# ARM-software/astc-encoder

Measured on AMD Instinct MI355X. Metric: Mtexels/s + PSNR-dB, 8192x8192 RGBA8 LDR 6x6 -medium, higher is better.
Workload: dtype f32

## Files before the change

astc-encoder_amd/csrc/astc_tables.h:

```cpp
#pragma once
#if !defined(__HIPCC_RTC__)
#include <stdint.h>
#include <stddef.h>
#else
typedef unsigned char uint8_t; typedef signed char int8_t; typedef unsigned short uint16_t; typedef short int16_t;
typedef unsigned int uint32_t; typedef int int32_t; typedef unsigned long uint64_t; typedef long int64_t;
typedef unsigned long size_t; typedef unsigned long uintptr_t; typedef long ptrdiff_t;
#define offsetof(type, member) __builtin_offsetof(type, member)
#endif

#if defined(__HIPCC__)
	#define ASTC_HD __host__ __device__
#else
	#define ASTC_HD
#endif

namespace astcd {

constexpr int MAX_TEXELS       = 216;
constexpr int MAX_WEIGHTS      = 64;
constexpr int PLANE2_OFFSET    = 32;
constexpr int MAX_PARTITIONS   = 4;
constexpr int MAX_PARTITIONINGS = 1024;
constexpr int MAX_KMEANS_TEXELS = 64;
constexpr int MAX_BLOCK_MODES  = 2048;
constexpr int MAX_DECIMATION_MODES = 87;
constexpr int MAX_TRIAL_CANDIDATES = 8;
constexpr int MAX_PARTITIONING_CANDIDATES = 8;
constexpr int MAX_ANGULAR_QUANT = 7;
constexpr int ANGULAR_STEPS = 32;
constexpr int SINCOS_STEPS  = 64;
constexpr float ERROR_CALC_DEFAULT = 1e30f;

enum {
	FMT_LUMINANCE = 0, FMT_LUMINANCE_DELTA = 1, FMT_HDR_LUMINANCE_LARGE_RANGE = 2,
	FMT_HDR_LUMINANCE_SMALL_RANGE = 3, FMT_LUMINANCE_ALPHA = 4, FMT_LUMINANCE_ALPHA_DELTA = 5,
	FMT_RGB_SCALE = 6, FMT_HDR_RGB_SCALE = 7, FMT_RGB = 8, FMT_RGB_DELTA = 9,
	FMT_RGB_SCALE_ALPHA = 10, FMT_HDR_RGB = 11, FMT_RGBA = 12, FMT_RGBA_DELTA = 13,
	FMT_HDR_RGB_LDR_ALPHA = 14, FMT_HDR_RGBA = 15
};

enum {
	QUANT_2 = 0, QUANT_3, QUANT_4, QUANT_5, QUANT_6, QUANT_8, QUANT_10, QUANT_12, QUANT_16,
	QUANT_20, QUANT_24, QUANT_32, QUANT_40, QUANT_48, QUANT_64, QUANT_80, QUANT_96, QUANT_128,
	QUANT_160, QUANT_192, QUANT_256
};

constexpr uint32_t MODE_DESC_BYTES = 16 + 2 * 32;
constexpr uint32_t MODE_WEIGHT_BYTES = 68;
constexpr uint32_t MODE_Q2U_BYTES = 12 * 32;
constexpr uint32_t FMT_QUANT_ROWS = 17;
ASTC_HD inline uint32_t fmt_comb_cols(uint32_t partition_limit) { return partition_limit <= 1 ? 0u : partition_limit == 2 ? 7u : partition_limit == 3 ? 10u : 13u; }
ASTC_HD inline uint32_t fmt_scratch_bytes(uint32_t partition_limit)
{
	uint32_t P = partition_limit < 1 ? 1u : partition_limit > 4 ? 4u : partition_limit;
	return P * FMT_QUANT_ROWS * 4 * 4 + P * FMT_QUANT_ROWS * 4 + FMT_QUANT_ROWS * fmt_comb_cols(P) * (4 + 2);
}
constexpr uint32_t ANG_PAIR_STRIDE = 9;
ASTC_HD inline uint32_t uni_region_bytes(uint32_t texel_count, uint32_t partition_limit)
{
	const uint32_t Tp = (texel_count + 3u) & ~3u;
	uint32_t bytes = 64 * ANG_PAIR_STRIDE * 4;
	if (8u * (MODE_DESC_BYTES + 64u + Tp * 4) > bytes) bytes = 8u * (MODE_DESC_BYTES + 64u + Tp * 4);
	if (fmt_scratch_bytes(partition_limit) > bytes) bytes = fmt_scratch_bytes(partition_limit);
	if (5 * Tp * 4 > bytes) bytes = 5 * Tp * 4;
	return (bytes + 15u) & ~15u;
}

enum { SYM_BTYPE_ERROR = 0, SYM_BTYPE_CONST_F16 = 1, SYM_BTYPE_CONST_U16 = 2, SYM_BTYPE_NONCONST = 3 };

struct BlockMode {
	uint16_t mode_index;
	uint8_t  decimation_mode;
	uint8_t  quant_mode;
	uint8_t  weight_bits;
	uint8_t  is_dual_plane;
	uint8_t  pad[2];
};

struct ModeStatic {
	uint32_t tw_off;
	uint32_t tcf_off;
	uint16_t dwi_off[2];
	uint16_t lh_off[2];
	uint8_t  taps;
	uint8_t  weights;
	uint8_t  quant_mode;
	uint8_t  weight_bits;
	uint8_t  is_dual_plane;
	uint8_t  pad[3];
};

struct DecimationMode {
	int8_t   maxprec_1plane;
	int8_t   maxprec_2planes;
	uint16_t refprec_1plane;
	uint16_t refprec_2planes;
	uint16_t dwi_offset[3];
	uint16_t lowhigh_offset[3];
};

struct DwiTap8 { uint32_t w[4]; };
struct DwiSlot {
	uint32_t wt_off;
	uint32_t wc_off;
	uint16_t refprec;
	uint8_t  weight_count;
	uint8_t  taps;
	uint8_t  flags;
	uint8_t  dm;
	uint8_t  set;
	uint8_t  index;
};

constexpr int DWI_MAX_CHUNKS = 15;
struct DwiOrderDir {
	uint32_t list_off;
	uint16_t chunk_start[DWI_MAX_CHUNKS + 1];
	uint16_t chunks;
	uint16_t pad;
};

struct InfillSet {
	uint32_t tw_off;
	uint32_t tcf_off;
	uint16_t dwi_offset;
	uint16_t refprec;
	uint8_t  taps;
	uint8_t  direct;
	uint8_t  dm;
	uint8_t  plane;
};

struct DecimationInfo {
	uint8_t  texel_count;
	uint8_t  weight_count;
	uint8_t  max_texel_weight_count;
	uint8_t  weight_x;
	uint8_t  weight_y;
	uint8_t  max_weight_texel_count;
	uint8_t  realign_levels;
	uint8_t  realign_slots;
	uint32_t off_texel_weights;
	uint32_t off_texel_contribs_int;
	uint32_t off_texel_contribs_f;
	uint32_t off_weight_texel_count;
	uint32_t off_weight_texels;
	uint32_t off_weight_contribs;
	uint32_t off_texel_contrib_for_weight;
	uint32_t off_realign_order;
	uint32_t off_realign_counts;
	uint32_t table_bytes;
	uint32_t off_realign_later;
	uint32_t realign_speculative;
	uint32_t pad[2];
};
static_assert(sizeof(DecimationInfo) == 64, "DecimationInfo is staged as one 64-byte record");
constexpr int REALIGN_LATER_MAX = 16;
#ifndef ASTC_REALIGN_SPEC_MIN
#define ASTC_REALIGN_SPEC_MIN 2
#endif
constexpr int REALIGN_SPECULATIVE_MIN_LEVELS = ASTC_REALIGN_SPEC_MIN;

struct PartitionHeader {
	uint16_t partition_index;
	uint8_t  partition_count;
	uint8_t  pad;
	uint8_t  texel_count[4];
};

struct QuantXfer {
	uint8_t  quant_to_unquant[32];
	uint8_t  scramble_map[32];
	uint16_t prev_next_values[65];
	uint16_t pad;
};

constexpr uint32_t CTX_CONFIG_BACK = 256;
constexpr uint32_t CTX_LAYOUT_BACK = 1024;

struct TableRoot {
	uint8_t  dim_x, dim_y, texel_count, dim_z;
	uint32_t block_mode_count_1plane_always;
	uint32_t block_mode_count_1plane_selected;
	uint32_t block_mode_count_1plane_2plane_selected;
	uint32_t decimation_mode_count_always;
	uint32_t decimation_mode_count_selected;
	uint32_t partitioning_count_selected[4];
	uint32_t partition_stride;
	uint32_t off_block_modes;
	uint32_t off_decimation_modes;
	uint32_t off_decimation_infos;
	uint32_t off_partitions[4];
	uint32_t off_coverage[4];
	uint32_t off_kmeans_texels;
	uint32_t off_color_unquant_to_uquant;
	uint32_t off_color_uquant_to_pquant;
	uint32_t off_quant_xfer;
	uint32_t off_quant_mode_table;
	uint32_t off_quant_mode_by_bits;
	uint32_t off_mode_levels;
	uint32_t off_integer_of_trits;
	uint32_t off_integer_of_quints;
	uint32_t off_sin_table;
	uint32_t off_cos_table;
	uint32_t off_cos_sin_table;
	uint32_t off_dm_by_weights;
	uint32_t off_mode_static;
	uint32_t max_decimation_table_bytes;
	uint32_t max_weight_texel_rows;
	uint32_t realign_rt_floats;
	uint32_t max_weights[2];
	uint32_t dwi_total_floats[2];
	uint32_t off_dwi_owner[2];
	uint32_t off_dwi_slots[2];
	uint32_t off_infill_sets[2];
	uint32_t dwi_sets[2];
	uint32_t dwi_used_sets[2][12];
	uint32_t lowhigh_floats[2];
	uint32_t off_dwi_order[2];
	uint32_t dwi_sets_per_chunk;
	uint32_t max_partitionings;
	uint32_t total_bytes;
};

struct DeviceConfig {
	int32_t  profile;
	uint32_t flags;
	float    cw[4];
	float    rgbm_m_scale;
	uint32_t tune_partition_count_limit;
	uint32_t tune_partition_index_limit[3];
	uint32_t tune_refinement_limit;
	uint32_t tune_candidate_limit;
	uint32_t tune_partitioning_candidate_limit[3];
	float    tune_db_limit;
	float    tune_mse_overshoot;
	float    tune_partition_early_out_limit_factor[2];
	float    tune_2plane_early_out_limit_correlation;
	float    tune_search_mode0_enable;
	uint32_t debug_dup_stage;
};

struct ImageDesc {
	const void* data;
	uint32_t dim_x, dim_y;
	uint32_t data_type;
	uint32_t swz[4];
	uint32_t blocks_x, blocks_y;
	uint32_t use_fast_load;
	const float* alpha_avg;
	uint32_t a_scale_radius;
	uint32_t dim_z, blocks_z;
	uint32_t fast_load_slice0;
	const uint32_t* list;
};

struct ImageSetEntryDesc {
	ImageDesc img;
	uint8_t* out;
};

}
```

astc-encoder_amd/csrc/backend.h:

```cpp
#pragma once
#include <stddef.h>
#include <stdint.h>
#include <atomic>
#include <vector>
#include "astc_tables.h"
#include "image_set.h"
#include "mip_filter.h"
#include "mip_post.h"

namespace astcd {

struct Backend;

struct CompressJob {
	const void* const* host_slices;
	const void* device_data;
	uint32_t dim_x, dim_y, dim_z;
	uint32_t data_type;
	uint32_t swz[4];
	uint8_t* host_out;
	uint8_t* device_out;
	void*    stream;
	float*   kernel_ms;
	uint32_t a_scale_radius;
	const std::atomic<int>* cancel_flag;
	void (*progress)(float);
	uint32_t fast_load_slice0;
	uint32_t halo_above, halo_below;
	const uint32_t* device_list;
	uint32_t list_count;
};

struct DecompressJob {
	const uint8_t* host_blocks;
	size_t   block_bytes;
	void* const* host_slices;
	uint32_t dim_x, dim_y, dim_z;
	uint32_t data_type;
	uint32_t swz[4];
};

struct DecompressDeviceJob {
	const uint8_t* device_blocks;
	void*    device_image;
	uint32_t dim_x, dim_y, dim_z;
	uint32_t data_type;
	uint32_t swz[4];
	void*    stream;
};

inline size_t texel_bytes(uint32_t data_type) { return data_type == 0 ? 4 : data_type == 1 ? 8 : 16; }

struct BlockGrid {
	uint32_t x, y, z;
	uint32_t dim_z;
	size_t count() const { return (size_t)x * y * z; }
};
template <class Job> inline BlockGrid block_grid(const TableRoot& root, const Job& job)
{
	const uint32_t dim_z = job.dim_z ? job.dim_z : 1u;
	return { (job.dim_x + root.dim_x - 1) / root.dim_x, (job.dim_y + root.dim_y - 1) / root.dim_y, (dim_z + root.dim_z - 1) / root.dim_z, dim_z };
}

inline bool uses_fast_load(const TableRoot& root, int32_t profile, const CompressJob& job)
{
	const bool identity = job.swz[0] == 0 && job.swz[1] == 1 && job.swz[2] == 2 && job.swz[3] == 3;
	return identity && profile < 2 && job.data_type == 0 && root.dim_z == 1;
}

inline ImageDesc image_desc(const TableRoot& root, int32_t profile, const CompressJob& job, const void* data)
{
	const BlockGrid g = block_grid(root, job);
	ImageDesc img;
	img.data = data;
	img.dim_x = job.dim_x; img.dim_y = job.dim_y; img.dim_z = g.dim_z;
	img.data_type = job.data_type;
	for (int i = 0; i < 4; i++) img.swz[i] = job.swz[i];
	img.blocks_x = g.x; img.blocks_y = g.y; img.blocks_z = g.z;
	img.use_fast_load = uses_fast_load(root, profile, job) ? 1 : 0;
	img.fast_load_slice0 = job.fast_load_slice0;
	img.alpha_avg = nullptr;
	img.a_scale_radius = job.a_scale_radius;
	img.list = job.device_list;
	return img;
}

struct CompressSetJob {
	const CompressJob* entries;
	uint32_t count;
	void*    stream;
	float*   kernel_ms;
	const std::atomic<int>* cancel_flag;
	void (*progress)(float);
	const struct MipChainJob* generate;
};

struct MipChainJob {
	const void* device_image;
	uint32_t dim_x, dim_y, dim_z, kind, data_type, level_count;
	uint32_t srgb;
	uint8_t* device_levels;
	size_t texels_offset[MIP_MAX_LEVELS];
	void* stream;
	uint32_t post_flags;
	float alpha_cutoff;
	uint32_t cover_t;
	float cover_hi, cover_lo;
	uint32_t filter_kind, filter_edge;
	uint32_t weight;
};

struct ResizeJob {
	const void* device_image;
	void* device_out;
	uint32_t dim_x, dim_y, dim_z, out_x, out_y, out_z, kind, data_type, srgb;
	uint32_t filter_kind, filter_edge, weight;
	void* stream;
	float* kernel_ms;
};

struct DecompressSetJob {
	const DecompressDeviceJob* entries;
	uint32_t count;
	void*    stream;
};

struct CompareJob {
	const void* device_a; uint32_t type_a;
	const void* device_b; uint32_t type_b;
	size_t texels;
	void* stream;
	double* sums;
	int hdr, fstop_lo, fstop_hi;
};
constexpr int METRIC_SUMS_HOST = 18;

struct QualityEntryJob {
	DecompressDeviceJob decode;
	const void* device_original; uint32_t original_type;
	double* device_block_errors;
};
struct QualitySetJob {
	const QualityEntryJob* entries;
	uint32_t count;
	void* stream;
	double* sums;
	int hdr, fstop_lo, fstop_hi;
};

Backend* backend_create(const uint8_t* blob, size_t blob_bytes, const DeviceConfig& cfg, int* status);
void backend_destroy(Backend* b);
int backend_device_count(const Backend* b);
int backend_compress(Backend* b, const CompressJob& job);
int backend_decompress(Backend* b, const DecompressJob& job);
int backend_decompress_device(Backend* b, const DecompressDeviceJob& job);
int backend_compare(Backend* b, const CompareJob& job);
int backend_compress_set(Backend* b, const CompressSetJob& job);
int backend_decompress_set(Backend* b, const DecompressSetJob& job);
int backend_compare_blocks_set(Backend* b, const QualitySetJob& job);
struct SelectJob {
	const double* device_block_errors;
	uint32_t dim_x, dim_y, dim_z;
	uint32_t blocks;
	double weight[4], max_mse;
	uint32_t* device_list;
	void* stream;
	uint32_t* count;
};
struct AdaptiveJob {
	CompressJob strong;
	DecompressDeviceJob decode;
	double weight[4], max_mse;
	double* device_block_errors;
	uint32_t* selected; uint32_t* replaced;
	float* kernel_ms_strong; float* kernel_ms_other;
};
int backend_select_blocks(Backend* b, const SelectJob& job);
int backend_adaptive_reserve(Backend* b, const void* device_image, const void* device_out, const void* device_block_errors, size_t blocks);
int backend_adaptive_refine(Backend* b, const AdaptiveJob& job);
int backend_generate_mips(Backend* b, const MipChainJob& job);
int backend_resize(Backend* b, const ResizeJob& job);
void backend_log(const char* fmt, ...) __attribute__((format(printf, 1, 2)));
const char* backend_name();
void backend_set_log_callback(void (*callback)(const char* message));


struct KernelLaunch {
	const uint8_t* d_tab;
	uint32_t lds_bytes;
	ImageDesc img;
	uint8_t* d_out;
	uint32_t first, count;
	void* stream;
	unsigned long long* d_prof;
	const ImageSetTable* d_set;
};

int astc_kernel_prepare_ldr(const TableRoot& root, const DeviceConfig& cfg, uint32_t* lds_bytes, void* layout_out, uint32_t* layout_bytes);
int astc_kernel_prepare_hdr(const TableRoot& root, const DeviceConfig& cfg, uint32_t* lds_bytes, void* layout_out, uint32_t* layout_bytes);
int astc_kernel_launch_ldr(const KernelLaunch& k);
int astc_kernel_launch_hdr(const KernelLaunch& k);
int astc_kernel_prepare_ldr64(const TableRoot& root, const DeviceConfig& cfg, uint32_t* lds_bytes, void* layout_out, uint32_t* layout_bytes);
int astc_kernel_prepare_hdr64(const TableRoot& root, const DeviceConfig& cfg, uint32_t* lds_bytes, void* layout_out, uint32_t* layout_bytes);
int astc_kernel_launch_ldr64(const KernelLaunch& k);
int astc_kernel_launch_hdr64(const KernelLaunch& k);
constexpr int ASTC_PREPARE_NOT_THIS_CONTEXT = -1;
#define ASTC_DECLARE_KERNEL_VARIANT(tag) \
	int astc_kernel_prepare_##tag(const TableRoot& root, const DeviceConfig& cfg, uint32_t* lds_bytes, void* layout_out, uint32_t* layout_bytes); \
	int astc_kernel_launch_##tag(const KernelLaunch& k);
ASTC_DECLARE_KERNEL_VARIANT(ldr_6x6m)
ASTC_DECLARE_KERNEL_VARIANT(ldr_8x8t)
ASTC_DECLARE_KERNEL_VARIANT(hdr_6x6m)
#undef ASTC_DECLARE_KERNEL_VARIANT
const char* backend_kernel_name(const Backend* b);
int backend_specialize(Backend* b);

constexpr size_t ALPHA_LDS_LIMIT = 160u * 1024u;
constexpr uint32_t ALPHA_TILE_ROWS_2D = 32;
struct AlphaLaunch {
	const void* d_image;
	float* d_averages;
	uint32_t dim_x, dim_y, dim_z, data_type, swz_a, radius;
	float* d_scratch; uint32_t scratch_workgroups;
	void* stream;
};
size_t astc_alpha_scratch_bytes(uint32_t dim_x, uint32_t dim_y, uint32_t dim_z, uint32_t radius, uint32_t* workgroups);
int astc_alpha_launch(const AlphaLaunch& a);

struct DecodeLaunch {
	const uint8_t* d_blocks;
	void* d_image;
	const void* d_tables;
	uint32_t dim_x, dim_y, dim_z, data_type, swz[4];
	uint32_t block_x, block_y, block_z, profile;
	void* stream;
};
int astc_decode_launch(const DecodeLaunch& d);
size_t astc_decode_set_bytes(uint32_t count);
uint32_t astc_decode_set_build(void* out, const DecodeLaunch* entries, uint32_t count);
int astc_decode_set_launch(const void* d_table, uint32_t runs, void* stream);
size_t astc_decode_tables_bytes();
void astc_decode_tables_build(void* out, uint32_t block_x, uint32_t block_y, uint32_t block_z);

struct QualityLaunch {
	DecodeLaunch decode;
	const void* d_original; uint32_t original_type;
	double* d_block_errors;
};
size_t astc_quality_set_bytes(uint32_t count);
size_t astc_quality_scratch_doubles();
uint32_t astc_quality_set_build(void* out, const QualityLaunch* entries, uint32_t count);
int astc_quality_set_launch(const void* h_table, const void* d_table, double* d_partials, double* d_sums, int hdr, int fstop_lo, int fstop_hi, void* stream);

struct SelectLaunch {
	const double* d_errors;
	uint32_t dim_x, dim_y, dim_z, block_x, block_y, block_z, blocks;
	double weight[4], max_mse;
	uint32_t* d_list;
	uint32_t* d_counts;
	void* stream;
};
size_t astc_select_scratch_words(size_t blocks);
size_t astc_select_total_word(size_t blocks);
int astc_select_launch(const SelectLaunch& s);
struct MergeLaunch {
	const uint32_t* d_list; const uint32_t* d_count;
	uint32_t blocks;
	uint32_t max_count;
	const double* d_strong_errors; double* d_base_errors;
	const uint8_t* d_strong; uint8_t* d_out;
	double weight[4];
	uint32_t* d_replaced;
	void* stream;
};
int astc_merge_launch(const MergeLaunch& m);

int astc_mip_launch(const MipChainJob& job, const void* d_srgb, void* stream);
size_t astc_mip_srgb_table_bytes();
void astc_mip_srgb_tables_build(void* out);
int astc_mip_weighted_launch(const MipChainJob& job, const void* d_srgb, void* stream);
int astc_mip_filter_table_build(const MipChainJob& job, std::vector<uint8_t>& out);
int astc_mip_filter_launch(const MipChainJob& job, const void* d_table, const void* d_srgb, void* stream);
int astc_mip_filter_weighted_launch(const MipChainJob& job, const void* d_table, const void* d_srgb, void* stream);
int astc_mip_cube_launch(const MipChainJob& job, const void* d_table, const void* d_srgb, void* stream);
size_t astc_mip_post_scratch_bytes(const MipChainJob& job);
int astc_mip_post_launch(const MipChainJob& job, void* d_scratch, void* stream);

int astc_resize_table_build(const ResizeJob& job, std::vector<uint8_t>& out);
int astc_resize_launch(const ResizeJob& job, const void* d_table, const void* d_srgb, void* stream);

struct CompareLaunch {
	const void* d_a; uint32_t type_a;
	const void* d_b; uint32_t type_b;
	size_t texels;
	double* d_sums;
	void* stream;
	int hdr, fstop_lo, fstop_hi;
};
int astc_compare_launch(const CompareLaunch& c);
size_t astc_compare_scratch_doubles();

}
```

astc-encoder_amd/csrc/backend_hip.hip:

```cpp
#include "backend.h"
#include "kernel_jit.h"
#include "mip_resample.h"

#include <hip/hip_runtime.h>
#include <chrono>
#include <cstdarg>
#include <cstdio>
#include <sched.h>
#include <atomic>
#include <cstdlib>
#include <cstring>
#include <condition_variable>
#include <functional>
#include <mutex>
#include <new>
#include <thread>
#include <type_traits>
#include <utility>
#include <vector>

namespace astcd {

struct SlotWorker {
	std::mutex mu;
	std::mutex state_mu;
	std::condition_variable wake, done_cv;
	std::function<void()> task;
	bool has_task = false, done = true, quit = false, bound = false;
	std::thread thread;
	bool started = false;
};

struct DeviceSlot {
	int device = 0;
	uint8_t* d_base = nullptr;
	uint8_t* d_tab = nullptr;
	uint8_t* d_dectab = nullptr;
	const double* d_srgb = nullptr;
	hipStream_t stream = nullptr;
	hipStream_t copy_stream = nullptr;
	hipEvent_t ev0 = nullptr, ev1 = nullptr, ev_copy[2] = {}, ev_band = nullptr, ev_done[3] = {}, ev_out[2] = {};
	hipEvent_t ev_gen = nullptr;
	uint8_t* h_in[2] = {}; size_t h_in_cap = 0;
	uint8_t* h_out[2] = {}; size_t h_out_cap = 0;
	void* d_image = nullptr; size_t image_cap = 0;
	uint8_t* d_out = nullptr; size_t out_cap = 0;
	float* d_alpha = nullptr; size_t alpha_cap = 0;
	float* d_alpha_scratch = nullptr; size_t alpha_scratch_cap = 0;
	uint8_t* d_mip_post = nullptr; size_t mip_post_cap = 0;
	uint8_t* d_mip_filter = nullptr; size_t mip_filter_cap = 0;
	std::vector<uint8_t> h_mip_filter;
	uint8_t* d_set = nullptr; size_t set_cap = 0;
	std::vector<uint8_t> h_set;
	unsigned long long* d_prof = nullptr;
	size_t trace_cap = 0;
	double* d_sums = nullptr;
	double* d_quality = nullptr; size_t quality_cap = 0;
	double* d_quality_sums = nullptr; size_t quality_sums_cap = 0;
	uint32_t* d_select = nullptr; size_t select_cap = 0;
	uint8_t* d_adaptive = nullptr; size_t adaptive_cap = 0;
	hipEvent_t ev_adapt[2] = {};
	std::mutex busy;
	std::vector<int> local_cpus;
	SlotWorker* worker = nullptr;
	hipModule_t jit_module = nullptr;
	hipFunction_t jit_fn = nullptr;
	bool jit_tried = false;
};

struct Backend {
	std::vector<DeviceSlot*> slots;
	std::vector<DeviceSlot*> extra;
	std::mutex slots_mu;
	std::vector<uint8_t> full;
	size_t dectab_offset;
	size_t srgb_offset;
	DeviceConfig cfg;
	uint32_t lds_bytes;
	bool hdr;
	TableRoot root;
	int variant;
	JitKernel* jit;
	JitMode jit_mode;
	std::atomic<unsigned long long> blocks_done;
	unsigned long long jit_lazy_blocks;
	std::atomic<bool> jit_active;
};

constexpr size_t ALLOC_SLACK = 4096;
constexpr size_t BAND_MIN_BLOCKS = (size_t)1 << 18;
#if defined(ASTC_TRACE)
constexpr size_t TRACE_WORDS_PER_BLOCK_HOST = 1024;
#endif

static std::atomic<void (*)(const char*)> g_log_callback{nullptr};
void backend_set_log_callback(void (*cb)(const char*)) { g_log_callback.store(cb); }
static void log_msg(const char* fmt, ...) __attribute__((format(printf, 1, 2)));
static void log_msg(const char* fmt, ...)
{
	void (*cb)(const char*) = g_log_callback.load();
	static const bool to_stderr = []() { const char* e = getenv("ASTCENC_AMD_LOG"); return e && strcmp(e, "stderr") == 0; }();
	if (!cb && !to_stderr) return;
	char line[512];
	va_list ap;
	va_start(ap, fmt);
	vsnprintf(line, sizeof(line), fmt, ap);
	va_end(ap);
	if (cb) cb(line);
	else fprintf(stderr, "astcenc_amd: %s\n", line);
}

void backend_log(const char* fmt, ...)
{
	char line[512];
	va_list ap;
	va_start(ap, fmt);
	vsnprintf(line, sizeof(line), fmt, ap);
	va_end(ap);
	log_msg("%s", line);
}

#define HIP_TRY(expr, fail) do { hipError_t e_ = (expr); if (e_ != hipSuccess) { \
	log_msg("%s -> %s", #expr, hipGetErrorString(e_)); fail; } } while (0)

const char* backend_name() { return "hip:gfx950"; }

namespace {

struct DeviceGuard {
	int saved; bool ok;
	DeviceGuard() : saved(0), ok(hipGetDevice(&saved) == hipSuccess) {}
	~DeviceGuard() { if (ok) (void)hipSetDevice(saved); }
};

template <class T> int grow(T*& buf, size_t& cap, size_t need)
{
	if (cap >= need) return 0;
	if (buf) (void)hipFree(buf);
	buf = nullptr; cap = 0;
	HIP_TRY(hipMalloc(reinterpret_cast<void**>(&buf), need + ALLOC_SLACK), return 1);
	cap = need;
	return 0;
}
int grow_pinned(uint8_t* (&pair)[2], size_t& cap, size_t need)
{
	if (cap >= need) return 0;
	for (uint8_t*& h : pair) { if (h) (void)hipHostFree(h); h = nullptr; }
	cap = 0;
	for (uint8_t*& h : pair) HIP_TRY(hipHostMalloc(reinterpret_cast<void**>(&h), need, hipHostMallocDefault), return 1);
	cap = need;
	return 0;
}

struct KernelVariant {
	const char* name;
	bool fixed, hdr, small;
	int (*prepare)(const TableRoot&, const DeviceConfig&, uint32_t*, void*, uint32_t*);
	int (*launch)(const KernelLaunch&);
};
const KernelVariant kernel_variants[] = {
	{ "astc_compress_blocks_ldr_6x6m", true, false, true, astc_kernel_prepare_ldr_6x6m, astc_kernel_launch_ldr_6x6m },
	{ "astc_compress_blocks_ldr_8x8t", true, false, true, astc_kernel_prepare_ldr_8x8t, astc_kernel_launch_ldr_8x8t },
	{ "astc_compress_blocks_hdr_6x6m", true, true, true, astc_kernel_prepare_hdr_6x6m, astc_kernel_launch_hdr_6x6m },
	{ "astc_compress_blocks_ldr64", false, false, true, astc_kernel_prepare_ldr64, astc_kernel_launch_ldr64 },
	{ "astc_compress_blocks_hdr64", false, true, true, astc_kernel_prepare_hdr64, astc_kernel_launch_hdr64 },
	{ "astc_compress_blocks_ldr", false, false, false, astc_kernel_prepare_ldr, astc_kernel_launch_ldr },
	{ "astc_compress_blocks_hdr", false, true, false, astc_kernel_prepare_hdr, astc_kernel_launch_hdr },
};
int kernel_prepare(Backend* b, uint32_t* lds_bytes, void* layout_out, uint32_t* layout_bytes)
{
	if (b->variant >= 0) return kernel_variants[b->variant].prepare(b->root, b->cfg, lds_bytes, layout_out, layout_bytes);
	const bool small = b->root.texel_count <= 64;
	const char* want = getenv("ASTCENC_AMD_KERNEL");
	const bool generic_only = want && strcmp(want, "generic") == 0;
	for (int i = 0; i < (int)(sizeof(kernel_variants) / sizeof(kernel_variants[0])); i++)
	{
		const KernelVariant& v = kernel_variants[i];
		if (v.hdr != b->hdr || v.small != small || (v.fixed && generic_only)) continue;
		const int rc = v.prepare(b->root, b->cfg, lds_bytes, layout_out, layout_bytes);
		if (rc == ASTC_PREPARE_NOT_THIS_CONTEXT) continue;
		if (rc == 0) b->variant = i;
		return rc;
	}
	return (int)hipErrorInvalidDeviceFunction;
}
int kernel_launch(const Backend* b, const DeviceSlot* s, const KernelLaunch& k)
{
	if (s->jit_fn)
	{
		KernelLaunch a = k;
		void* args[] = { &a.d_tab, &a.img, &a.d_out, &a.first, &a.count, &a.d_prof, &a.d_set };
		return (int)hipModuleLaunchKernel(s->jit_fn, k.count, 1, 1, 64, 1, 1, k.lds_bytes, static_cast<hipStream_t>(k.stream), args, nullptr);
	}
	return kernel_variants[b->variant].launch(k);
}

bool jit_self_check(Backend* b, DeviceSlot* s, hipFunction_t fn)
{
	const uint32_t bsx = b->root.dim_x, bsy = b->root.dim_y, bsz = b->root.dim_z;
	const uint32_t nbx = bsz > 1 ? 16u : 48u, nby = bsz > 1 ? 16u : 48u, nbz = bsz > 1 ? 8u : 1u;
	const uint32_t dim_x = nbx * bsx - 1u, dim_y = nby * bsy - 1u, dim_z = bsz > 1 ? nbz * bsz - 1u : 1u;
	const size_t texels = (size_t)dim_x * dim_y * dim_z, nblocks = (size_t)nbx * nby * nbz;
	std::vector<uint8_t> img(texels * 4);
	uint32_t rng = 0x9E3779B1u;
	auto tri = [](uint32_t v) { const uint32_t m = v & 511u; return (int)(m < 256u ? m : 511u - m); };
	for (uint32_t z = 0; z < dim_z; z++)
		for (uint32_t y = 0; y < dim_y; y++)
			for (uint32_t x = 0; x < dim_x; x++)
			{
				const uint32_t tile = (x / bsx + 3u * (y / bsy) + 5u * (z / bsz) + y / (3u * bsy)) % 9u;
				uint8_t* px = &img[(((size_t)z * dim_y + y) * dim_x + x) * 4];
				int grey = 0;
				for (int ch = 0; ch < 4; ch++)
				{
					rng = rng * 1664525u + 1013904223u;
					const int noise = (int)(rng >> 24);
					int v = (int)((x * (3u + ch) + y * (7u - ch) + z * 11u) & 255u);
					if (tile == 1) v += (noise & 15) - 6;
					else if (tile == 2) v += (noise & 63) - 24;
					else if (tile == 3) v = noise;
					else if (tile == 4) v = ((x + ch) ^ (y >> 1)) & 2 ? 220 - 20 * ch : 30 + 25 * ch;
					else if (tile == 5) v = 40 + 50 * ch;
					else if (tile == 6 || tile == 7)
					{
						if (ch == 0) grey = (3 * tri(x + 2u * y + 5u * z) + tri((3u * x + 512u - y) >> 1)) / 4 + noise % 21 - 10;
						v = ch < 3 ? grey : 192 + tri((x >> 1) + (y >> 2)) / 4 + noise % 7 - 3;
					}
					else if (tile == 8) v = tri(x * (2u + ch) + y * (5u - ch) + z * 3u);
					if (ch == 3 && tile != 3 && tile != 2 && tile != 7) v = 255;
					px[ch] = (uint8_t)(v < 0 ? 0 : v > 255 ? 255 : v);
				}
			}
	void* d_img = nullptr;
	uint8_t* d_out = nullptr;
	bool ok = hipMalloc(&d_img, img.size() + ALLOC_SLACK) == hipSuccess && hipMalloc(reinterpret_cast<void**>(&d_out), 2 * nblocks * 16 + ALLOC_SLACK) == hipSuccess;
	std::vector<uint8_t> out(2 * nblocks * 16);
	if (ok)
	{
		CompressJob job;
		memset(&job, 0, sizeof(job));
		job.dim_x = dim_x; job.dim_y = dim_y; job.dim_z = dim_z;
		for (int i = 0; i < 4; i++) job.swz[i] = (uint32_t)i;
		KernelLaunch k;
		k.d_tab = s->d_tab; k.lds_bytes = b->lds_bytes; k.d_prof = nullptr; k.d_set = nullptr; k.stream = s->stream;
		k.first = 0; k.count = (uint32_t)nblocks;
		k.img = image_desc(b->root, b->cfg.profile, job, d_img);
		ok = hipMemcpyAsync(d_img, img.data(), img.size(), hipMemcpyHostToDevice, s->stream) == hipSuccess;
		k.d_out = d_out;
		ok = ok && kernel_variants[b->variant].launch(k) == 0;
		k.d_out = d_out + nblocks * 16;
		void* args[] = { &k.d_tab, &k.img, &k.d_out, &k.first, &k.count, &k.d_prof, &k.d_set };
		ok = ok && hipModuleLaunchKernel(fn, k.count, 1, 1, 64, 1, 1, k.lds_bytes, s->stream, args, nullptr) == hipSuccess;
		ok = ok && hipMemcpyAsync(out.data(), d_out, out.size(), hipMemcpyDeviceToHost, s->stream) == hipSuccess;
		ok = ok && hipStreamSynchronize(s->stream) == hipSuccess;
		if (!ok) (void)hipGetLastError();
	}
	if (d_img) (void)hipFree(d_img);
	if (d_out) (void)hipFree(d_out);
	return ok && memcmp(out.data(), out.data() + nblocks * 16, nblocks * 16) == 0;
}

void slot_adopt_jit(Backend* b, DeviceSlot* s)
{
	if (!b->jit || s->jit_tried || jit_state(b->jit) != JIT_READY) return;
	s->jit_tried = true;
	size_t bytes = 0;
	const void* code = jit_code(b->jit, &bytes);
	hipModule_t mod = nullptr;
	hipFunction_t fn = nullptr;
	if (hipModuleLoadData(&mod, code) != hipSuccess || hipModuleGetFunction(&fn, mod, JIT_ENTRY_POINT) != hipSuccess)
	{
		(void)hipGetLastError();
		if (mod) (void)hipModuleUnload(mod);
		log_msg("run-time build %s does not load on device %d: the generic build stays", jit_kernel_name(b->jit), s->device);
		return;
	}
	const char* check = getenv("ASTCENC_AMD_JIT_SELF_CHECK");
	if (!(check && strcmp(check, "0") == 0) && !jit_self_check(b, s, fn))
	{
		(void)hipModuleUnload(mod);
		log_msg("run-time build %s does not reproduce the generic build's bytes on the self-check image: the generic build stays", jit_kernel_name(b->jit));
		return;
	}
	s->jit_module = mod;
	s->jit_fn = fn;
	b->jit_active.store(true);
}

void worker_stop(SlotWorker* w)
{
	if (!w) return;
	if (w->started)
	{
		{ std::lock_guard<std::mutex> g(w->state_mu); w->quit = true; }
		w->wake.notify_one();
		w->thread.join();
	}
	delete w;
}

void slot_destroy(DeviceSlot* s)
{
	if (!s) return;
	worker_stop(s->worker);
	s->worker = nullptr;
	(void)hipSetDevice(s->device);
	if (s->d_image) (void)hipFree(s->d_image);
	if (s->d_out) (void)hipFree(s->d_out);
	if (s->d_alpha) (void)hipFree(s->d_alpha);
	if (s->d_alpha_scratch) (void)hipFree(s->d_alpha_scratch);
	if (s->d_mip_post) (void)hipFree(s->d_mip_post);
	if (s->d_mip_filter) (void)hipFree(s->d_mip_filter);
	if (s->d_set) (void)hipFree(s->d_set);
	if (s->d_sums) (void)hipFree(s->d_sums);
	if (s->d_quality) (void)hipFree(s->d_quality);
	if (s->d_quality_sums) (void)hipFree(s->d_quality_sums);
	if (s->d_select) (void)hipFree(s->d_select);
	if (s->d_adaptive) (void)hipFree(s->d_adaptive);
	for (hipEvent_t e : s->ev_adapt) if (e) (void)hipEventDestroy(e);
	if (s->d_prof) (void)hipFree(s->d_prof);
	for (int i = 0; i < 2; i++) { if (s->h_in[i]) (void)hipHostFree(s->h_in[i]); if (s->h_out[i]) (void)hipHostFree(s->h_out[i]); }
	for (hipEvent_t e : { s->ev_copy[0], s->ev_copy[1], s->ev_band, s->ev_done[0], s->ev_done[1], s->ev_done[2], s->ev_out[0], s->ev_out[1], s->ev0, s->ev1, s->ev_gen })
		if (e) (void)hipEventDestroy(e);
	if (s->copy_stream) (void)hipStreamDestroy(s->copy_stream);
	if (s->stream) (void)hipStreamDestroy(s->stream);
	if (s->jit_module) (void)hipModuleUnload(s->jit_module);
	if (s->d_base) (void)hipFree(s->d_base);
	delete s;
}

static std::vector<int> device_local_cpus(int device)
{
	std::vector<int> cpus;
	char bus[64] = { 0 };
	if (hipDeviceGetPCIBusId(bus, (int)sizeof(bus), device) != hipSuccess) return cpus;
	for (char* p = bus; *p; p++) if (*p >= 'A' && *p <= 'F') *p = (char)(*p - 'A' + 'a');
	char path[160];
	snprintf(path, sizeof(path), "/sys/bus/pci/devices/%s/local_cpulist", bus);
	FILE* f = fopen(path, "r");
	if (!f) return cpus;
	char line[1024] = { 0 };
	if (fgets(line, (int)sizeof(line), f))
	{
		for (char* p = line; *p && *p != '\n'; )
		{
			char* end = nullptr;
			long a = strtol(p, &end, 10);
			if (end == p) break;
			long bnd = a;
			p = end;
			if (*p == '-') { bnd = strtol(p + 1, &end, 10); p = end; }
			for (long c = a; c <= bnd && c < 4096; c++) cpus.push_back((int)c);
			if (*p == ',') p++;
		}
	}
	fclose(f);
	return cpus;
}

static void bind_worker_to_device(const DeviceSlot* s)
{
	static const bool enabled = []() { const char* e = getenv("ASTCENC_AMD_NUMA_BIND"); return !(e && e[0] == '0'); }();
	if (!enabled || s->local_cpus.empty()) return;
	cpu_set_t allowed, want;
	CPU_ZERO(&want);
	if (sched_getaffinity(0, sizeof(allowed), &allowed) != 0) return;
	int n = 0;
	for (int c : s->local_cpus) if (c < CPU_SETSIZE && CPU_ISSET(c, &allowed)) { CPU_SET(c, &want); n++; }
	if (n > 0) (void)sched_setaffinity(0, sizeof(want), &want);
}

static bool worker_run(DeviceSlot* s, std::function<void()> task)
{
	SlotWorker* w = s->worker;
	if (!w) return false;
	if (!w->mu.try_lock()) return false;
	if (!w->started)
	{
		try
		{
			w->thread = std::thread([w, s]()
			{
				bind_worker_to_device(s);
				std::unique_lock<std::mutex> lk(w->state_mu);
				for (;;)
				{
					w->wake.wait(lk, [w]() { return w->has_task || w->quit; });
					if (w->quit) return;
					std::function<void()> t = std::move(w->task);
					w->has_task = false;
					lk.unlock();
					t();
					lk.lock();
					w->done = true;
					w->done_cv.notify_all();
				}
			});
			w->started = true;
		}
		catch (...) { w->mu.unlock(); return false; }
	}
	{
		std::lock_guard<std::mutex> g(w->state_mu);
		w->task = std::move(task);
		w->has_task = true;
		w->done = false;
	}
	w->wake.notify_one();
	return true;
}
static void worker_wait(DeviceSlot* s)
{
	SlotWorker* w = s->worker;
	{
		std::unique_lock<std::mutex> lk(w->state_mu);
		w->done_cv.wait(lk, [w]() { return w->done; });
	}
	w->mu.unlock();
}

DeviceSlot* slot_create(Backend* b, int device, int* status)
{
	DeviceSlot* s = new DeviceSlot();
	s->device = device;
#define SLOT_TRY(expr, code) HIP_TRY(expr, { slot_destroy(s); *status = code; return nullptr; })
	SLOT_TRY(hipSetDevice(device), 2);
	{
		uint8_t layout[CTX_LAYOUT_BACK - CTX_CONFIG_BACK]; uint32_t layout_bytes = 0, lds_bytes = 0;
		int prc = kernel_prepare(b, &lds_bytes, layout, &layout_bytes);
		if (prc != 0)
		{
			log_msg("kernel setup failed on device %d (hip error %d)", device, prc);
			slot_destroy(s); *status = 2; return nullptr;
		}
	}
	SLOT_TRY(hipMalloc(&s->d_base, b->full.size() + ALLOC_SLACK), 1);
	SLOT_TRY(hipMemcpy(s->d_base, b->full.data(), b->full.size(), hipMemcpyHostToDevice), 2);
	s->d_tab = s->d_base + CTX_LAYOUT_BACK;
	s->d_dectab = s->d_base + b->dectab_offset;
	s->d_srgb = reinterpret_cast<const double*>(s->d_base + b->srgb_offset);
	SLOT_TRY(hipStreamCreateWithFlags(&s->stream, hipStreamNonBlocking), 2);
	SLOT_TRY(hipStreamCreateWithFlags(&s->copy_stream, hipStreamNonBlocking), 2);
	SLOT_TRY(hipEventCreateWithFlags(&s->ev_copy[0], hipEventDisableTiming), 2);
	SLOT_TRY(hipEventCreateWithFlags(&s->ev_copy[1], hipEventDisableTiming), 2);
	SLOT_TRY(hipEventCreateWithFlags(&s->ev_band, hipEventDisableTiming), 2);
	for (int i = 0; i < 3; i++) SLOT_TRY(hipEventCreateWithFlags(&s->ev_done[i], hipEventDisableTiming), 2);
	for (int i = 0; i < 2; i++) SLOT_TRY(hipEventCreateWithFlags(&s->ev_out[i], hipEventDisableTiming), 2);
	SLOT_TRY(hipEventCreate(&s->ev0), 2);
	SLOT_TRY(hipEventCreate(&s->ev1), 2);
	SLOT_TRY(hipEventCreate(&s->ev_gen), 2);
#if defined(ASTC_PROFILE)
	enum { PS_COUNT = 40 };
	SLOT_TRY(hipMalloc(&s->d_prof, 2 * PS_COUNT * sizeof(unsigned long long)), 1);
	SLOT_TRY(hipMemset(s->d_prof, 0, 2 * PS_COUNT * sizeof(unsigned long long)), 2);
#endif
#undef SLOT_TRY
	s->local_cpus = device_local_cpus(device);
	slot_adopt_jit(b, s);
	*status = 0;
	return s;
}

std::vector<int> device_list(int ndev)
{
	std::vector<int> out;
	const char* env = getenv("ASTCENC_AMD_DEVICES");
	const bool all = env && strcmp(env, "all") == 0;
	if (env && *env && !all)
	{
		const char* p = env;
		while (*p)
		{
			char* e = nullptr;
			long v = strtol(p, &e, 10);
			if (e == p) break;
			if (v >= 0 && v < ndev) out.push_back((int)v);
			else log_msg("ASTCENC_AMD_DEVICES names device %ld, %d visible; ignored", v, ndev);
			p = e;
			while (*p == ',' || *p == ' ') p++;
		}
	}
	if (out.empty())
	{
		int cur = 0;
		if (hipGetDevice(&cur) != hipSuccess) cur = 0;
		out.push_back(cur);
		if (all) for (int d = 0; d < ndev; d++) if (d != cur) out.push_back(d);
	}
	return out;
}

DeviceSlot* slot_for_pointer(Backend* b, const void* ptr, int* status)
{
	*status = 0;
	hipPointerAttribute_t attr;
	memset(&attr, 0, sizeof(attr));
	if (!ptr || hipPointerGetAttributes(&attr, ptr) != hipSuccess)
	{
		(void)hipGetLastError();
		return b->slots[0];
	}
	for (DeviceSlot* s : b->slots) if (s->device == attr.device) return s;
	std::lock_guard<std::mutex> lk(b->slots_mu);
	for (DeviceSlot* s : b->extra) if (s->device == attr.device) return s;
	DeviceSlot* s = slot_create(b, attr.device, status);
	if (s) b->extra.push_back(s);
	return s;
}

bool pick_stream(const DeviceSlot* s, void* caller_stream, hipStream_t* out)
{
	*out = s->stream;
	if (!caller_stream) return true;
	hipStream_t stream = static_cast<hipStream_t>(caller_stream);
	hipDevice_t sdev = -1;
	if (hipStreamGetDevice(stream, &sdev) != hipSuccess) { (void)hipGetLastError(); sdev = s->device; }
	if ((int)sdev != s->device)
	{
		log_msg("the stream belongs to device %d, the buffers to device %d", (int)sdev, s->device);
		return false;
	}
	*out = stream;
	return true;
}

bool set_on_one_device(const DeviceSlot* s, const void* const* ptrs, size_t count)
{
	for (size_t i = 0; i < count; i++)
	{
		hipPointerAttribute_t attr;
		memset(&attr, 0, sizeof(attr));
		if (!ptrs[i] || hipPointerGetAttributes(&attr, ptrs[i]) != hipSuccess) { (void)hipGetLastError(); continue; }
		if (attr.device != s->device)
		{
			log_msg("image set entry %zu: a buffer of device %d, entry 0's are on device %d", i / 2, attr.device, s->device);
			return false;
		}
	}
	return true;
}

template <class Body> int run_locked(DeviceSlot* s, void* caller_stream, Body body)
{
	std::lock_guard<std::mutex> busy(s->busy);
	HIP_TRY(hipSetDevice(s->device), return 2);
	hipStream_t stream;
	if (!pick_stream(s, caller_stream, &stream)) return 3;
	return body(s, stream);
}

template <class Body> int run_on_owner(Backend* b, const void* owner, const void* const* same_device, size_t count, void* caller_stream, Body body)
{
	DeviceGuard guard;
	int st = 0;
	DeviceSlot* s = slot_for_pointer(b, owner, &st);
	if (!s) return st ? st : 2;
	if (!set_on_one_device(s, same_device, count)) return 3;
	return run_locked(s, caller_stream, body);
}

template <class Job> DecodeLaunch decode_launch(const Backend* b, const DeviceSlot* s, const Job& job, const uint8_t* d_blocks, void* d_image, hipStream_t stream)
{
	DecodeLaunch d;
	d.d_blocks = d_blocks;
	d.d_image = d_image;
	d.d_tables = s->d_dectab;
	d.dim_x = job.dim_x; d.dim_y = job.dim_y; d.dim_z = job.dim_z ? job.dim_z : 1u; d.data_type = job.data_type;
	for (int i = 0; i < 4; i++) d.swz[i] = job.swz[i];
	d.block_x = b->root.dim_x; d.block_y = b->root.dim_y; d.block_z = b->root.dim_z;
	d.profile = b->cfg.profile;
	d.stream = stream;
	return d;
}

struct Progress {
	std::mutex mu;
	size_t done, total;
	void (*callback)(float);
	void add(size_t n)
	{
		if (!callback) return;
		std::lock_guard<std::mutex> lk(mu);
		done += n;
		callback(100.0f * (float)done / (float)total);
	}
};

}

Backend* backend_create(const uint8_t* blob, size_t blob_bytes, const DeviceConfig& cfg, int* status)
{
	int ndev = 0;
	if (hipGetDeviceCount(&ndev) != hipSuccess || ndev == 0)
	{
		log_msg("no HIP device available; this library has no CPU fallback");
		*status = 2;
		return nullptr;
	}
	DeviceGuard guard;

	Backend* b = new Backend;
	b->cfg = cfg;
	memcpy(&b->root, blob, sizeof(TableRoot));
	b->hdr = cfg.profile >= 2;
	b->lds_bytes = 0;
	b->variant = -1;
	b->jit = nullptr; b->jit_mode = JIT_OFF; b->blocks_done.store(0); b->jit_active.store(false);
	b->jit_lazy_blocks = JIT_LAZY_BLOCKS;
	if (const char* e = getenv("ASTCENC_AMD_JIT_LAZY_BLOCKS")) { const long long v = strtoll(e, nullptr, 10); if (v >= 1) b->jit_lazy_blocks = (unsigned long long)v; }
	uint8_t layout[CTX_LAYOUT_BACK - CTX_CONFIG_BACK];
	uint32_t layout_bytes = 0;
	{
		int prc = kernel_prepare(b, &b->lds_bytes, layout, &layout_bytes);
		if (prc != 0)
		{
			log_msg("kernel setup failed (hip error %d)", prc);
			delete b; *status = 2; return nullptr;
		}
	}
	if (b->lds_bytes > 160 * 1024)
	{
		log_msg("block working set %u B; a CU has 160 KiB of LDS", b->lds_bytes);
		delete b; *status = 2; return nullptr;
	}

	b->dectab_offset = (CTX_LAYOUT_BACK + blob_bytes + 255) & ~(size_t)255;
	b->srgb_offset = (b->dectab_offset + astc_decode_tables_bytes() + 255) & ~(size_t)255;
	b->full.assign(b->srgb_offset + astc_mip_srgb_table_bytes(), 0);
	astc_decode_tables_build(b->full.data() + b->dectab_offset, b->root.dim_x, b->root.dim_y, b->root.dim_z);
	astc_mip_srgb_tables_build(b->full.data() + b->srgb_offset);
	memcpy(b->full.data(), layout, layout_bytes);
	static_assert(sizeof(DeviceConfig) <= 256, "DeviceConfig outgrew its slot");
	memcpy(b->full.data() + (CTX_LAYOUT_BACK - CTX_CONFIG_BACK), &b->cfg, sizeof(DeviceConfig));
	memcpy(b->full.data() + CTX_LAYOUT_BACK, blob, blob_bytes);

#if !defined(ASTC_TRACE) && !defined(ASTC_DUPSTAGE) && !defined(ASTC_PROFILE) && !defined(ASTC_LDS_PAD_ENV)
	{
		const char* want = getenv("ASTCENC_AMD_KERNEL");
		b->jit_mode = want && strcmp(want, "generic") == 0 ? JIT_OFF : jit_mode_from_environment();
		if (b->jit_mode != JIT_OFF && !kernel_variants[b->variant].fixed)
		{
			int dev = 0;
			hipDeviceProp_t prop;
			if (hipGetDevice(&dev) == hipSuccess && hipGetDeviceProperties(&prop, dev) == hipSuccess)
				b->jit = jit_acquire(layout, layout_bytes, b->cfg, b->root, b->hdr, prop.gcnArchName, [](const char* line) { log_msg("%s", line); });
			if (b->jit && b->jit_mode == JIT_EAGER) jit_start(b->jit);
			if (b->jit && b->jit_mode == JIT_SYNC) (void)jit_wait(b->jit);
		}
	}
#endif
	for (int device : device_list(ndev))
	{
		int st = 0;
		DeviceSlot* s = slot_create(b, device, &st);
		if (!s)
		{
			if (b->slots.empty()) { jit_release(b->jit); delete b; *status = st; return nullptr; }
			log_msg("device %d not usable, continuing with %zu device(s)", device, b->slots.size());
			continue;
		}
		if (!b->slots.empty()) s->worker = new (std::nothrow) SlotWorker();
		b->slots.push_back(s);
	}
	*status = 0;
	return b;
}

void backend_destroy(Backend* b)
{
	if (!b) return;
	DeviceGuard guard;
	for (DeviceSlot* s : b->slots) slot_destroy(s);
	for (DeviceSlot* s : b->extra) slot_destroy(s);
	jit_release(b->jit);
	delete b;
}

int backend_device_count(const Backend* b) { return (int)b->slots.size(); }
const char* backend_kernel_name(const Backend* b)
{
	if (b->jit && b->jit_active.load()) return jit_kernel_name(b->jit);
	return b->variant >= 0 ? kernel_variants[b->variant].name : "";
}

int backend_specialize(Backend* b)
{
	if (b->variant >= 0 && kernel_variants[b->variant].fixed) return 0;
	if (!b->jit || jit_wait(b->jit) != JIT_READY) return 1;
	DeviceGuard guard;
	for (DeviceSlot* s : b->slots)
	{
		std::lock_guard<std::mutex> busy(s->busy);
		if (hipSetDevice(s->device) == hipSuccess) slot_adopt_jit(b, s);
	}
	return b->jit_active.load() ? 0 : 1;
}

static void jit_count_blocks(Backend* b, DeviceSlot* s, size_t nblocks)
{
	slot_adopt_jit(b, s);
	if (b->jit && b->jit_mode == JIT_LAZY && b->blocks_done.fetch_add(nblocks) + nblocks >= b->jit_lazy_blocks) jit_start(b->jit);
}

static int alpha_prepass(DeviceSlot* s, hipStream_t stream, const void* d_image, float* d_averages, uint32_t dim_x, uint32_t rows,
                         uint32_t dim_z, uint32_t data_type, uint32_t swz_a, uint32_t radius)
{
	AlphaLaunch a;
	a.d_image = d_image; a.d_averages = d_averages;
	a.dim_x = dim_x; a.dim_y = rows; a.dim_z = dim_z; a.data_type = data_type;
	a.swz_a = swz_a; a.radius = radius; a.stream = stream;
	a.d_scratch = nullptr; a.scratch_workgroups = 0;
	const size_t scratch = astc_alpha_scratch_bytes(dim_x, rows, dim_z, radius, &a.scratch_workgroups);
	if (scratch == (size_t)-1)
	{
		log_msg("a_scale_radius %u needs more than 1 GiB of pre-pass scratch per tile: refused", radius);
		return 1;
	}
	if (scratch)
	{
		if (grow(s->d_alpha_scratch, s->alpha_scratch_cap, scratch) != 0) return 1;
		a.d_scratch = s->d_alpha_scratch;
	}
	int arc = astc_alpha_launch(a);
	if (arc != 0) { log_msg("alpha pre-pass launch failed (hip error %d)", arc); return 2; }
	return 0;
}

static void alpha_scratch_release(DeviceSlot* s, hipStream_t stream)
{
	if (s->alpha_scratch_cap > ((size_t)64 << 20))
	{
		(void)hipStreamSynchronize(stream);
		(void)hipFree(s->d_alpha_scratch);
		s->d_alpha_scratch = nullptr; s->alpha_scratch_cap = 0;
	}
}

struct ChunkLoop {
	KernelLaunch k;
	size_t nblocks, chunk;
	bool chunked;
	bool timed;
	const std::atomic<int>* cancel_flag;
	Progress* progress;
	std::function<int(size_t first, size_t n)> before_launch;
	std::function<int(size_t first, size_t n, size_t chunk_index, size_t prev_blocks)> after_launch;
	size_t launched, prev_blocks;
};

static int run_chunks(const Backend* b, DeviceSlot* s, ChunkLoop& L)
{
	const hipStream_t stream = static_cast<hipStream_t>(L.k.stream);
	if (L.timed) HIP_TRY(hipEventRecord(s->ev0, stream), return 2);
	L.launched = 0; L.prev_blocks = 0;
	size_t chunk_index = 0;
	for (size_t first = 0; first < L.nblocks; first += L.chunk, chunk_index++)
	{
		if (L.cancel_flag && L.cancel_flag->load(std::memory_order_relaxed)) break;
		size_t n = L.nblocks - first < L.chunk ? L.nblocks - first : L.chunk;
		if (L.before_launch && L.before_launch(first, n) != 0) return 2;
		KernelLaunch k = L.k;
		k.first = (uint32_t)first; k.count = (uint32_t)n;
		int lrc = kernel_launch(b, s, k);
		if (lrc != 0) { log_msg("kernel launch failed (hip error %d)", lrc); return 2; }
		L.launched = first + n;
		if (L.after_launch)
		{
			if (L.after_launch(first, n, chunk_index, L.prev_blocks) != 0) return 2;
		}
		else if (L.chunked)
		{
			HIP_TRY(hipEventRecord(s->ev_done[chunk_index % 3], stream), return 2);
			if (chunk_index > 0)
			{
				HIP_TRY(hipEventSynchronize(s->ev_done[(chunk_index - 1) % 3]), return 2);
				if (L.progress) L.progress->add(L.prev_blocks);
			}
		}
		L.prev_blocks = n;
	}
	if (L.timed) HIP_TRY(hipEventRecord(s->ev1, stream), return 2);
	return 0;
}

static int compress_pipeline(Backend* b, DeviceSlot* s, hipStream_t stream, const CompressJob& job, Progress* progress);

static int compress_on_slot(Backend* b, DeviceSlot* s, hipStream_t stream, const CompressJob& job, Progress* progress)
{
	const int rc = compress_pipeline(b, s, stream, job, progress);
	if (rc != 0)
	{
		(void)hipStreamSynchronize(s->copy_stream);
		(void)hipStreamSynchronize(s->stream);
	}
	return rc;
}

static int compress_pipeline(Backend* b, DeviceSlot* s, hipStream_t stream, const CompressJob& job, Progress* progress)
{
	const BlockGrid grid = block_grid(b->root, job);
	const uint32_t bsy = b->root.dim_y, dim_z = grid.dim_z, blocks_x = grid.x, blocks_y = grid.y;
	const size_t nblocks = job.device_list ? (size_t)job.list_count : grid.count();
	jit_count_blocks(b, s, nblocks);
	const size_t row_bytes = (size_t)job.dim_x * texel_bytes(job.data_type);
	const uint32_t halo_above = dim_z == 1 && job.a_scale_radius != 0 ? job.halo_above : 0u;
	const uint32_t halo_below = dim_z == 1 && job.a_scale_radius != 0 ? job.halo_below : 0u;
	const uint32_t rows_with_halo = job.dim_y + halo_above + halo_below;
	const size_t slice_bytes = rows_with_halo * row_bytes;
	const size_t image_bytes = slice_bytes * dim_z;
	const size_t out_bytes = grid.count() * 16;

	const void* d_image = job.device_data;
	uint8_t* d_out = job.device_out;

	if (job.host_slices)
	{
		if (grow(s->d_image, s->image_cap, image_bytes) != 0) return 1;
		d_image = s->d_image;
	}
	const bool banded = job.host_slices && job.host_out && dim_z == 1 && job.a_scale_radius == 0;
	if (job.host_slices && !banded)
	{
		for (uint32_t z = 0; z < dim_z; z++)
			HIP_TRY(hipMemcpyAsync(static_cast<uint8_t*>(s->d_image) + z * slice_bytes, job.host_slices[z], slice_bytes, hipMemcpyHostToDevice, stream), return 2);
	}
	if (job.host_out)
	{
		if (grow(s->d_out, s->out_cap, out_bytes) != 0) return 1;
		d_out = s->d_out;
	}
	if (!d_image || !d_out) return 2;

	ImageDesc img = image_desc(b->root, b->cfg.profile, job, static_cast<const uint8_t*>(d_image) + halo_above * row_bytes);
	if (job.a_scale_radius != 0)
	{
		if (grow(s->d_alpha, s->alpha_cap, (size_t)job.dim_x * rows_with_halo * sizeof(float)) != 0) return 1;
		const int arc = alpha_prepass(s, stream, d_image, s->d_alpha, job.dim_x, rows_with_halo, dim_z, job.data_type, job.swz[3], job.a_scale_radius);
		if (arc != 0) return arc;
		img.alpha_avg = s->d_alpha + (size_t)halo_above * job.dim_x;
		alpha_scratch_release(s, stream);
	}

	const bool chunked = (progress && progress->callback) || job.host_slices;
	size_t chunk = chunked ? (size_t)1 << 18 : nblocks;
	if (banded)
	{
		size_t rows = chunk / blocks_x;
		if (rows * 4 > blocks_y) rows = nblocks >= BAND_MIN_BLOCKS ? (blocks_y + 3) / 4 : blocks_y;
		if (rows < 1) rows = 1;
		chunk = rows * blocks_x;
	}
	if (banded)
	{
		const size_t band_rows = (chunk / blocks_x) * bsy;
		if (grow_pinned(s->h_in, s->h_in_cap, band_rows * row_bytes) != 0 || grow_pinned(s->h_out, s->h_out_cap, chunk * 16) != 0) return 1;
	}
	auto upload_band = [&](size_t band_first, size_t band_blocks) -> int {
		const size_t band = band_first / chunk;
		const size_t y0 = (band_first / blocks_x) * bsy;
		size_t y1 = ((band_first + band_blocks) / blocks_x) * bsy;
		if (y1 > job.dim_y) y1 = job.dim_y;
		if (band >= 2) HIP_TRY(hipEventSynchronize(s->ev_copy[band & 1]), return 2);
		memcpy(s->h_in[band & 1], static_cast<const uint8_t*>(job.host_slices[0]) + y0 * row_bytes, (y1 - y0) * row_bytes);
		HIP_TRY(hipMemcpyAsync(static_cast<uint8_t*>(s->d_image) + y0 * row_bytes, s->h_in[band & 1], (y1 - y0) * row_bytes, hipMemcpyHostToDevice, s->copy_stream), return 2);
		HIP_TRY(hipEventRecord(s->ev_copy[band & 1], s->copy_stream), return 2);
		return 0;
	};
	auto collect_band = [&](size_t band_first, size_t band_blocks) -> int {
		const size_t band = band_first / chunk;
		HIP_TRY(hipEventSynchronize(s->ev_out[band & 1]), return 2);
		memcpy(job.host_out + band_first * 16, s->h_out[band & 1], band_blocks * 16);
		if (progress) progress->add(band_blocks);
		return 0;
	};
#if defined(ASTC_TRACE)
	{
		const size_t need = grid.count() * TRACE_WORDS_PER_BLOCK_HOST * sizeof(uint32_t);
		if (grow(s->d_prof, s->trace_cap, need) != 0) return 1;
		HIP_TRY(hipMemsetAsync(s->d_prof, 0, need, stream), return 2);
	}
#endif
	ChunkLoop L;
	L.k.d_tab = s->d_tab; L.k.lds_bytes = b->lds_bytes; L.k.img = img; L.k.d_out = d_out;
	L.k.stream = stream; L.k.d_prof = s->d_prof; L.k.d_set = nullptr;
	L.nblocks = nblocks; L.chunk = chunk; L.chunked = chunked; L.timed = job.kernel_ms != nullptr;
	L.cancel_flag = job.cancel_flag; L.progress = progress;
	if (banded)
	{
		L.before_launch = [&](size_t first, size_t n) -> int {
			if (first == 0 && upload_band(0, n) != 0) return 2;
			const size_t next = first + n;
			if (next < nblocks && upload_band(next, nblocks - next < chunk ? nblocks - next : chunk) != 0) return 2;
			HIP_TRY(hipStreamWaitEvent(stream, s->ev_copy[(first / chunk) & 1], 0), return 2);
			return 0;
		};
		L.after_launch = [&](size_t first, size_t n, size_t chunk_index, size_t prev_blocks) -> int {
			HIP_TRY(hipEventRecord(s->ev_band, stream), return 2);
			HIP_TRY(hipStreamWaitEvent(s->copy_stream, s->ev_band, 0), return 2);
			HIP_TRY(hipMemcpyAsync(s->h_out[chunk_index & 1], d_out + first * 16, n * 16, hipMemcpyDeviceToHost, s->copy_stream), return 2);
			HIP_TRY(hipEventRecord(s->ev_out[chunk_index & 1], s->copy_stream), return 2);
			if (chunk_index > 0 && collect_band(first - prev_blocks, prev_blocks) != 0) return 2;
			return 0;
		};
	}
	if (run_chunks(b, s, L) != 0) return 2;
	const size_t launched = L.launched, prev_blocks = L.prev_blocks;

	if (job.host_out && !banded && launched)
	{
		HIP_TRY(hipMemcpyAsync(job.host_out, d_out, launched * 16, hipMemcpyDeviceToHost, stream), return 2);
	}
	HIP_TRY(hipStreamSynchronize(stream), return 2);
	if (banded)
	{
		if (launched && collect_band(launched - prev_blocks, prev_blocks) != 0) return 2;
		HIP_TRY(hipStreamSynchronize(s->copy_stream), return 2);
	}
	else if (chunked && progress && prev_blocks && launched) progress->add(prev_blocks);
	if (job.kernel_ms) HIP_TRY(hipEventElapsedTime(job.kernel_ms, s->ev0, s->ev1), return 2);
#if defined(ASTC_TRACE)
	if (const char* path = getenv("ASTCENC_AMD_TRACE_FILE"))
	{
		std::vector<uint32_t> host(grid.count() * TRACE_WORDS_PER_BLOCK_HOST);
		HIP_TRY(hipMemcpy(host.data(), s->d_prof, host.size() * sizeof(uint32_t), hipMemcpyDeviceToHost), return 2);
		if (FILE* f = fopen(path, "wb")) { fwrite(host.data(), sizeof(uint32_t), host.size(), f); fclose(f); }
	}
#endif
#if defined(ASTC_PROFILE)
	{
		enum { PS_COUNT = 40, PS_TOTAL = 14 };
		static const char* names[PS_COUNT] = { "load", "ideal", "decimate", "angular", "modes", "formats", "recompute", "pack", "diff",
		                                        "realign", "kmeans+partsearch", "  partscore", "physical", "stats", "TOTAL", "blocks",
		                                        "  dec sweep1", "  dec infill", "  dec sweep3", "  ang phase1", "  ang phase2",
		                                        "  mode terms", "  mode acc", "  mode quant", "  fmt eci", "  fmt table", "  fmt combine", "  fmt select",
		                                        "  cand staging", "  physical", "  refine (all)", "  trial (all)",
		                                        "  y0 cand quantize", "  y1 cand setup", "  y2 after pack", "  y3 accept/copy", "  y4 realign infill", "  y5 realign undecimated", "  y6 realign lane-per-weight eval", "  y7 realign movers" };
		unsigned long long h[2 * PS_COUNT];
		HIP_TRY(hipMemcpy(h, s->d_prof, sizeof(h), hipMemcpyDeviceToHost), return 2);
		HIP_TRY(hipMemset(s->d_prof, 0, sizeof(h)), return 2);
		fprintf(stderr, "stage cycles per block (lane-0 shader clock), %zu blocks:   [calls per block]\n", nblocks);
		for (int i = 0; i < PS_COUNT; i++)
			if (i != 15 && h[i])
				fprintf(stderr, "  %-18s %12.0f  %5.1f%%   [%6.2f]\n", names[i], (double)h[i] / (double)nblocks, 100.0 * (double)h[i] / (double)h[PS_TOTAL],
				        (double)h[PS_COUNT + i] / (double)nblocks);
	}
#endif
	return 0;
}

constexpr size_t MIN_BLOCKS_PER_DEVICE = 16384;
constexpr size_t DEAL_PORTIONS_PER_DEVICE = 4;
constexpr size_t MIN_BLOCKS_PER_PORTION = 4 * MIN_BLOCKS_PER_DEVICE;

static uint32_t shard_units(const BlockGrid& grid) { return grid.dim_z == 1 ? grid.y : grid.z; }

static size_t devices_for(const Backend* b, const BlockGrid& grid)
{
	size_t ndev = b->slots.size();
	const size_t by_size = grid.count() / MIN_BLOCKS_PER_DEVICE;
	if (ndev > by_size) ndev = by_size < 1 ? 1 : by_size;
	if (ndev > shard_units(grid)) ndev = shard_units(grid);
	return ndev;
}

static const void* advance(const void* p, size_t bytes) { return static_cast<const uint8_t*>(p) + bytes; }
static void* advance(void* p, size_t bytes) { return static_cast<uint8_t*>(p) + bytes; }

template <class Job> struct Shard {
	Job job;
	std::vector<std::decay_t<decltype(*std::declval<Job&>().host_slices)>> slices;
	uint32_t first_row;
	size_t first_block, blocks;
};

template <class Job> static std::vector<Shard<Job>> cut_shards(const Backend* b, const BlockGrid& grid, const Job& job, size_t count)
{
	const uint32_t units = shard_units(grid), units_per = (uint32_t)((units + count - 1) / count);
	const size_t unit_blocks = grid.dim_z == 1 ? (size_t)grid.x : (size_t)grid.x * grid.y;
	const size_t row_bytes = (size_t)job.dim_x * texel_bytes(job.data_type);
	std::vector<Shard<Job>> shards;
	for (uint32_t u0 = 0; u0 < units; u0 += units_per)
	{
		const uint32_t u1 = u0 + units_per < units ? u0 + units_per : units;
		Shard<Job> sh;
		sh.job = job;
		sh.first_row = 0;
		sh.first_block = u0 * unit_blocks;
		sh.blocks = (u1 - u0) * unit_blocks;
		if (grid.dim_z == 1)
		{
			const uint32_t y0 = u0 * b->root.dim_y;
			const uint32_t y1 = u1 * b->root.dim_y < job.dim_y ? u1 * b->root.dim_y : job.dim_y;
			sh.first_row = y0;
			sh.slices.push_back(advance(job.host_slices[0], y0 * row_bytes));
			sh.job.dim_y = y1 - y0;
		}
		else
		{
			const uint32_t z0 = u0 * b->root.dim_z;
			const uint32_t z1 = u1 * b->root.dim_z < grid.dim_z ? u1 * b->root.dim_z : grid.dim_z;
			sh.slices.assign(job.host_slices + z0, job.host_slices + z1);
			sh.job.dim_z = z1 - z0;
		}
		shards.push_back(std::move(sh));
	}
	for (Shard<Job>& sh : shards) sh.job.host_slices = sh.slices.data();
	return shards;
}

static int deal_portions(Backend* b, size_t ndev, size_t count, const std::function<int(DeviceSlot*, size_t)>& run, const char* log_as)
{
	std::vector<int> rcs(count, 0);
	std::atomic<size_t> next_portion{0};
	std::atomic<bool> failed{false};
	const size_t nslots = ndev < count ? ndev : count;
	std::vector<double> busy_ms(nslots, 0.0);
	std::vector<unsigned> taken(nslots, 0u);
	auto deal = [&](size_t g)
	{
		const auto t0 = std::chrono::steady_clock::now();
		for (;;)
		{
			if (failed.load()) break;
			const size_t p = next_portion.fetch_add(1);
			if (p >= count) break;
			rcs[p] = run(b->slots[g], p);
			if (rcs[p] != 0) failed.store(true);
			taken[g]++;
		}
		busy_ms[g] = std::chrono::duration<double, std::milli>(std::chrono::steady_clock::now() - t0).count();
	};
	std::vector<size_t> on_workers;
	for (size_t g = 1; g < nslots; g++)
	{
		try { if (worker_run(b->slots[g], [&deal, g]() { deal(g); })) on_workers.push_back(g); }
		catch (...) { }
	}
	deal(0);
	for (size_t g : on_workers) worker_wait(b->slots[g]);
	if (log_as)
		for (size_t g = 0; g < nslots; g++) log_msg("%s: device slot %zu took %u of %zu portions, busy %.2f ms", log_as, g, taken[g], count, busy_ms[g]);
	int rc = 0;
	for (int r : rcs) if (r != 0 && (rc == 0 || r == 1)) rc = r;
	return rc;
}

int backend_compress(Backend* b, const CompressJob& job)
{
	const BlockGrid grid = block_grid(b->root, job);
	Progress progress;
	progress.done = 0; progress.callback = job.progress; progress.total = job.device_list ? job.list_count : grid.count();

	const void* list_ptr[1] = { job.device_list };
	if (!job.host_slices)
		return run_on_owner(b, job.device_data, list_ptr, 1, job.stream, [&](DeviceSlot* s, hipStream_t stream) { return compress_on_slot(b, s, stream, job, &progress); });

	DeviceGuard guard;
	auto on_slot = [b, &progress](DeviceSlot* slot, const CompressJob& j)
	{
		return run_locked(slot, j.stream, [&](DeviceSlot* s, hipStream_t stream) { return compress_on_slot(b, s, stream, j, &progress); });
	};
	size_t ndev = (job.a_scale_radius != 0 && grid.dim_z > 1) || !job.host_out ? 1 : devices_for(b, grid);
#if defined(ASTC_TRACE)
	ndev = 1;
#endif
	if (ndev <= 1) return on_slot(b->slots[0], job);

// ... 447 lines not shown
```

astc-encoder_amd/csrc/kernel_device.h:

```cpp
#pragma once
#include "wave_block.h"
#include "image_set.h"

#ifndef ASTC_KERNEL_LINKAGE
#define ASTC_KERNEL_LINKAGE
#endif

#ifndef ASTC_WAVES_PER_EU
#define ASTC_WAVES_PER_EU 4
#endif

namespace astcd {

__device__ inline uint32_t xcd_block_remap(uint32_t b, uint32_t n)
{
	const uint32_t per = n / 8u;
	const uint32_t even = per * 8u;
	if (b >= even) return b;
	return (b % 8u) * per + (b / 8u);
}

constexpr uint32_t XCD_SET_RUN = 1024;
__device__ inline uint32_t xcd_block_remap_runs(uint32_t b, uint32_t n)
{
	const uint32_t group = XCD_SET_RUN * 8u;
	const uint32_t even = n / group * group;
	if (b >= even) return b;
	const uint32_t g = b / group, r = b - g * group;
	return g * group + (r % 8u) * XCD_SET_RUN + r / 8u;
}

ASTC_KERNEL_LINKAGE __global__ void __launch_bounds__(64, ASTC_WAVES_PER_EU) __attribute__((amdgpu_waves_per_eu(ASTC_WAVES_PER_EU)))
ASTC_KERNEL_NAME(const uint8_t* __restrict__ tab, ImageDesc img,
                 uint8_t* __restrict__ out, uint32_t first_block, uint32_t num_blocks, unsigned long long* prof,
                 const ImageSetTable* __restrict__ set)
{
	typedef const __attribute__((address_space(4))) uint8_t* constant_bytes;
	uint32_t b = (set ? xcd_block_remap_runs(blockIdx.x, num_blocks) : xcd_block_remap(blockIdx.x, num_blocks)) + first_block;
	if (img.list)
	{
		b = reinterpret_cast<const __attribute__((address_space(4))) uint32_t*>(reinterpret_cast<uintptr_t>(img.list))[b];
		if (b >= img.blocks_x * img.blocks_y * img.blocks_z) return;
	}
	uint8_t* lds = lds_base();
#if defined(ASTC_TRACE)
	const uint32_t trace_slot = b;
#endif
	if (set)
	{
		const constant_bytes t = (constant_bytes)reinterpret_cast<uintptr_t>(set);
		const uint32_t count = reinterpret_cast<const __attribute__((address_space(4))) ImageSetTable*>(t)->count;
		const __attribute__((address_space(4))) uint32_t* first =
			reinterpret_cast<const __attribute__((address_space(4))) uint32_t*>(t + image_set_first_offset());
		const uint32_t e = image_set_find(first, count, b);
		const ImageSetEntryDesc rec = image_set_record<ImageSetEntryDesc>(reinterpret_cast<const __attribute__((address_space(4))) uint32_t*>(
			t + image_set_records_offset(count) + (size_t)e * sizeof(ImageSetEntryDesc)));
		img = rec.img;
		out = rec.out;
		b -= first[e];
	}
	uint32_t row = b / img.blocks_x;
	uint32_t bx = b - row * img.blocks_x;
	uint32_t bz = img.blocks_z > 1 ? row / img.blocks_y : 0u;
	uint32_t by = row - bz * img.blocks_y;

	uintptr_t base_bits = reinterpret_cast<uintptr_t>(tab) - CTX_LAYOUT_BACK;
	asm volatile("" : "+s"(base_bits));
	const uint8_t* const base = (const uint8_t*)(constant_bytes)base_bits;
	tab = base + CTX_LAYOUT_BACK;
	Ctx c;
	c.tab = tab;
	c.tab_constant = true;
	c.lds = lds;
#if ASTC_FIXED
	c.root = &kFixedRoot;
	c.cfg = &kFixedConfig;
	c.L = &kFixedLayout;
#else
	c.root = reinterpret_cast<const TableRoot*>(tab);
	c.cfg = reinterpret_cast<const DeviceConfig*>(base + (CTX_LAYOUT_BACK - CTX_CONFIG_BACK));
	c.L = reinterpret_cast<const LdsLayout*>(base);
#endif
	c.T = (int)c.L->texel_count;
#if defined(ASTC_FIXED_OPAQUE_TEXEL_COUNT)
	c.T = wv_uniform(wv_opaque(c.T));
#endif
	c.Tp = (c.T + 3) & ~3;
	c.Ts = lds_row_stride(c.Tp);
#if defined(ASTC_TRACE)
	if (prof) prof = reinterpret_cast<unsigned long long*>(reinterpret_cast<uint32_t*>(prof) + (size_t)trace_slot * TRACE_WORDS_PER_BLOCK);
#endif
	c.prof = prof;

	WV_ONE
	{
		LdsHeader* h = reinterpret_cast<LdsHeader*>(lds);
		h->base = base;
		h->prof = prof;
		c.blk().block_index = b;
	}
	WV_SYNC();

	PROF_SCOPE(c, PS_TOTAL);
	{
		PROF_SCOPE(c, PS_LOAD);
		if (img.alpha_avg && !block_has_visible_alpha(c, img, bx, by)) load_transparent_block(c);
		else DUP_STAGE(c, DUP_LOAD, load_block(c, img, bx, by, bz));
	}
	compress_block(c, out);
}

}
```

astc-encoder_amd/csrc/kernel_hdr.hip:

```cpp
#define ASTC_VARIANT v_hdr
#define ASTC_ENABLE_HDR 1
#define ASTC_KERNEL_NAME astc_compress_blocks_hdr
#define ASTC_PREPARE_NAME astc_kernel_prepare_hdr
#define ASTC_LAUNCH_NAME astc_kernel_launch_hdr
#include "kernel_impl.h"
```

astc-encoder_amd/csrc/kernel_hdr64.hip:

```cpp
#define ASTC_VARIANT v_hdr64
#define ASTC_ENABLE_HDR 1
#define ASTC_TEXELS_LE_64 1
#define ASTC_KERNEL_NAME astc_compress_blocks_hdr64
#define ASTC_PREPARE_NAME astc_kernel_prepare_hdr64
#define ASTC_LAUNCH_NAME astc_kernel_launch_hdr64
#include "kernel_impl.h"
```

astc-encoder_amd/csrc/kernel_hdr_6x6m.hip:

```cpp
#define ASTC_VARIANT v_hdr_6x6m
#define ASTC_ENABLE_HDR 1
#define ASTC_TEXELS_LE_64 1
#define ASTC_FIXED_CONTEXT 1
#define ASTC_FIXED_hdr_6x6_medium 1
#define ASTC_KERNEL_NAME astc_compress_blocks_hdr_6x6m
#define ASTC_PREPARE_NAME astc_kernel_prepare_hdr_6x6m
#define ASTC_LAUNCH_NAME astc_kernel_launch_hdr_6x6m
#include "kernel_impl.h"
```

astc-encoder_amd/csrc/kernel_impl.h:

```cpp
#include "backend.h"
#include "kernel_device.h"
#include <hip/hip_runtime.h>
#include <cstring>
#include <cstdlib>

namespace astcd {

int ASTC_PREPARE_NAME(const TableRoot& root, const DeviceConfig& cfg, uint32_t* lds_bytes, void* layout_out, uint32_t* layout_bytes)
{
	LdsLayout L;
	make_lds_layout(root, cfg, L);
#if ASTC_FIXED
	{
		DeviceConfig live = cfg;
		live.debug_dup_stage = kFixedConfig.debug_dup_stage;
		if (memcmp(&L, &kFixedLayout, sizeof(L)) != 0 || memcmp(&live, &kFixedConfig, sizeof(live)) != 0 || memcmp(&root, &kFixedRoot, sizeof(root)) != 0)
			return ASTC_PREPARE_NOT_THIS_CONTEXT;
	}
#endif
	*lds_bytes = L.total;
	static_assert(sizeof(LdsLayout) <= CTX_LAYOUT_BACK - CTX_CONFIG_BACK, "layout record grew past the space the backend reserves");
	memcpy(layout_out, &L, sizeof(L));
	*layout_bytes = (uint32_t)sizeof(L);
	return (int)hipFuncSetAttribute(reinterpret_cast<const void*>(ASTC_KERNEL_NAME),
	                                hipFuncAttributeMaxDynamicSharedMemorySize, (int)L.total);
}

int ASTC_LAUNCH_NAME(const KernelLaunch& k)
{
#if defined(ASTC_LDS_PAD_ENV)
	static const unsigned pad = getenv("ASTC_LDS_PAD") ? (unsigned)atoi(getenv("ASTC_LDS_PAD")) : 0u;
	if (pad) (void)hipFuncSetAttribute(reinterpret_cast<const void*>(ASTC_KERNEL_NAME), hipFuncAttributeMaxDynamicSharedMemorySize, (int)(k.lds_bytes + pad));
	hipLaunchKernelGGL(ASTC_KERNEL_NAME, dim3(k.count), dim3(64), k.lds_bytes + pad, static_cast<hipStream_t>(k.stream),
	                   k.d_tab, k.img, k.d_out, k.first, k.count, k.d_prof, k.d_set);
	return (int)hipGetLastError();
#endif
	hipLaunchKernelGGL(ASTC_KERNEL_NAME, dim3(k.count), dim3(64), k.lds_bytes, static_cast<hipStream_t>(k.stream),
	                   k.d_tab, k.img, k.d_out, k.first, k.count, k.d_prof, k.d_set);
	return (int)hipGetLastError();
}

}
```

astc-encoder_amd/csrc/kernel_jit.cpp:

```cpp
#include "kernel_jit.h"
#include "wave_ctx.h"

#include <hip/hiprtc.h>
#include <dlfcn.h>
#include <fcntl.h>
#include <link.h>
#include <signal.h>
#include <spawn.h>
#include <sys/stat.h>
#include <sys/wait.h>
#include <unistd.h>
#include <atomic>
#include <cerrno>
#include <chrono>
#include <condition_variable>
#include <cstdio>
#include <cstdlib>
#include <cstring>
#include <deque>
#include <map>
#include <mutex>
#include <string>
#include <thread>
#include <vector>

#define ASTC_EMBED(sym, file) \
	__asm__(".pushsection .rodata\n" ".balign 16\n" #sym ":\n" ".incbin \"" file "\"\n" ".byte 0\n" #sym "_end:\n" ".popsection\n"); \
	extern "C" const char sym[]; extern "C" const char sym##_end[];
ASTC_EMBED(astc_src_kernel_device, "kernel_device.h")
ASTC_EMBED(astc_src_wave_block, "wave_block.h")
ASTC_EMBED(astc_src_wave, "wave.h")
ASTC_EMBED(astc_src_wave_ctx, "wave_ctx.h")
ASTC_EMBED(astc_src_astc_tables, "astc_tables.h")
ASTC_EMBED(astc_src_wave_quad, "wave_quad.h")
ASTC_EMBED(astc_src_wave_load, "wave_load.h")
ASTC_EMBED(astc_src_wave_ideal, "wave_ideal.h")
ASTC_EMBED(astc_src_wave_weights, "wave_weights.h")
ASTC_EMBED(astc_src_wave_format, "wave_format.h")
ASTC_EMBED(astc_src_wave_color, "wave_color.h")
ASTC_EMBED(astc_src_wave_color_hdr, "wave_color_hdr.h")
ASTC_EMBED(astc_src_wave_refine, "wave_refine.h")
ASTC_EMBED(astc_src_wave_batch, "wave_batch.h")
ASTC_EMBED(astc_src_wave_partition, "wave_partition.h")
ASTC_EMBED(astc_src_wave_pack, "wave_pack.h")
ASTC_EMBED(astc_src_image_set, "image_set.h")

extern char** environ;

namespace astcd {
namespace {

struct EmbeddedHeader { const char* name; const char* text; const char* end; };
const EmbeddedHeader kHeaders[] = {
	{ "kernel_device.h", astc_src_kernel_device, astc_src_kernel_device_end }, { "wave_block.h", astc_src_wave_block, astc_src_wave_block_end },
	{ "wave.h", astc_src_wave, astc_src_wave_end }, { "wave_ctx.h", astc_src_wave_ctx, astc_src_wave_ctx_end },
	{ "astc_tables.h", astc_src_astc_tables, astc_src_astc_tables_end }, { "wave_quad.h", astc_src_wave_quad, astc_src_wave_quad_end },
	{ "wave_load.h", astc_src_wave_load, astc_src_wave_load_end }, { "wave_ideal.h", astc_src_wave_ideal, astc_src_wave_ideal_end },
	{ "wave_weights.h", astc_src_wave_weights, astc_src_wave_weights_end }, { "wave_format.h", astc_src_wave_format, astc_src_wave_format_end },
	{ "wave_color.h", astc_src_wave_color, astc_src_wave_color_end }, { "wave_color_hdr.h", astc_src_wave_color_hdr, astc_src_wave_color_hdr_end },
	{ "wave_refine.h", astc_src_wave_refine, astc_src_wave_refine_end }, { "wave_batch.h", astc_src_wave_batch, astc_src_wave_batch_end },
	{ "wave_partition.h", astc_src_wave_partition, astc_src_wave_partition_end }, { "wave_pack.h", astc_src_wave_pack, astc_src_wave_pack_end },
	{ "image_set.h", astc_src_image_set, astc_src_image_set_end },
};
constexpr int kHeaderCount = (int)(sizeof(kHeaders) / sizeof(kHeaders[0]));
constexpr long JIT_MAX_SCRATCH_BYTES = 32;

struct Rtc {
	void* handle = nullptr;
	decltype(&hiprtcCreateProgram) create = nullptr;
	decltype(&hiprtcCompileProgram) compile = nullptr;
	decltype(&hiprtcGetCodeSize) code_size = nullptr;
	decltype(&hiprtcGetCode) code = nullptr;
	decltype(&hiprtcGetProgramLogSize) log_size = nullptr;
	decltype(&hiprtcGetProgramLog) log = nullptr;
	decltype(&hiprtcDestroyProgram) destroy = nullptr;
	decltype(&hiprtcVersion) version = nullptr;
	int major = 0, minor = 0;
	bool ok = false;
};
const Rtc& rtc()
{
	static const Rtc r = []() {
		Rtc t;
		const char* names[] = { getenv("ASTCENC_AMD_HIPRTC"), "libhiprtc.so.7", "libhiprtc.so", "/opt/rocm/lib/libhiprtc.so" };
		for (const char* n : names)
		{
			if (!n || !*n) continue;
			t.handle = dlopen(n, RTLD_NOW | RTLD_LOCAL);
			if (t.handle) break;
		}
		if (!t.handle) return t;
		t.create = reinterpret_cast<decltype(t.create)>(dlsym(t.handle, "hiprtcCreateProgram"));
		t.compile = reinterpret_cast<decltype(t.compile)>(dlsym(t.handle, "hiprtcCompileProgram"));
		t.code_size = reinterpret_cast<decltype(t.code_size)>(dlsym(t.handle, "hiprtcGetCodeSize"));
		t.code = reinterpret_cast<decltype(t.code)>(dlsym(t.handle, "hiprtcGetCode"));
		t.log_size = reinterpret_cast<decltype(t.log_size)>(dlsym(t.handle, "hiprtcGetProgramLogSize"));
		t.log = reinterpret_cast<decltype(t.log)>(dlsym(t.handle, "hiprtcGetProgramLog"));
		t.destroy = reinterpret_cast<decltype(t.destroy)>(dlsym(t.handle, "hiprtcDestroyProgram"));
		t.version = reinterpret_cast<decltype(t.version)>(dlsym(t.handle, "hiprtcVersion"));
		t.ok = t.create && t.compile && t.code_size && t.code && t.log_size && t.log && t.destroy;
		if (t.ok && t.version) (void)t.version(&t.major, &t.minor);
		return t;
	}();
	return r;
}

uint64_t fnv1a(uint64_t h, const void* data, size_t n)
{
	const uint8_t* p = static_cast<const uint8_t*>(data);
	for (size_t i = 0; i < n; i++) { h ^= p[i]; h *= 1099511628211ull; }
	return h;
}

std::string records_text(const LdsLayout& L, const DeviceConfig& cfg, const TableRoot& r)
{
	static_assert(sizeof(LdsLayout) % 4 == 0 && sizeof(TableRoot) % 4 == 0, "records are word arrays");
	static_assert(sizeof(DeviceConfig) == 92, "DeviceConfig changed: update records_text (and oracle/emu/backend_emu.cpp)");
	std::string s;
	char t[96];
	auto word = [&](uint32_t v) { snprintf(t, sizeof(t), "%uu", v); s += t; };
	auto flt = [&](float f) { uint32_t v; memcpy(&v, &f, 4); snprintf(t, sizeof(t), "__builtin_bit_cast(float, %uu)", v); s += t; };
	s += "constexpr LdsLayout kFixedLayout = { ";
	for (size_t i = 0; i < sizeof(LdsLayout) / 4; i++) { if (i) s += ", "; word(reinterpret_cast<const uint32_t*>(&L)[i]); }
	s += " };\nconstexpr DeviceConfig kFixedConfig = { ";
	snprintf(t, sizeof(t), "%d, ", (int)cfg.profile); s += t;
	word(cfg.flags); s += ", { ";
	for (int i = 0; i < 4; i++) { if (i) s += ", "; flt(cfg.cw[i]); }
	s += " }, "; flt(cfg.rgbm_m_scale); s += ", "; word(cfg.tune_partition_count_limit); s += ", { ";
	for (int i = 0; i < 3; i++) { if (i) s += ", "; word(cfg.tune_partition_index_limit[i]); }
	s += " }, "; word(cfg.tune_refinement_limit); s += ", "; word(cfg.tune_candidate_limit); s += ", { ";
	for (int i = 0; i < 3; i++) { if (i) s += ", "; word(cfg.tune_partitioning_candidate_limit[i]); }
	s += " }, "; flt(cfg.tune_db_limit); s += ", "; flt(cfg.tune_mse_overshoot); s += ", { ";
	flt(cfg.tune_partition_early_out_limit_factor[0]); s += ", "; flt(cfg.tune_partition_early_out_limit_factor[1]);
	s += " }, "; flt(cfg.tune_2plane_early_out_limit_correlation); s += ", "; flt(cfg.tune_search_mode0_enable); s += ", 0u };\n";
	snprintf(t, sizeof(t), "constexpr TableRoot kFixedRoot = { %u, %u, %u, %u", (unsigned)r.dim_x, (unsigned)r.dim_y, (unsigned)r.texel_count, (unsigned)r.dim_z);
	s += t;
	for (size_t i = 1; i < sizeof(TableRoot) / 4; i++) { s += ", "; word(reinterpret_cast<const uint32_t*>(&r)[i]); }
	s += " };\n";
	return s;
}

std::string cache_dir()
{
	const char* e = getenv("ASTCENC_AMD_CACHE_DIR");
	if (e) return *e ? std::string(e) : std::string();
	if ((e = getenv("XDG_CACHE_HOME")) && *e) return std::string(e) + "/astcenc_amd";
	if ((e = getenv("HOME")) && *e) return std::string(e) + "/.cache/astcenc_amd";
	return std::string();
}
void make_dirs(const std::string& path)
{
	for (size_t i = 1; i <= path.size(); i++)
		if (i == path.size() || path[i] == '/') (void)mkdir(path.substr(0, i).c_str(), 0755);
}


std::string helper_path()
{
	static const std::string path = []() {
		const char* e = getenv("ASTCENC_AMD_JITC");
		if (e) return std::string(e);
		Dl_info info;
		if (!dladdr(reinterpret_cast<const void*>(&helper_path), &info) || !info.dli_fname) return std::string();
		std::string p(info.dli_fname);
		const size_t slash = p.rfind('/');
		p = (slash == std::string::npos ? std::string(".") : p.substr(0, slash)) + "/astcenc_amd_jitc";
		return access(p.c_str(), X_OK) == 0 ? p : std::string();
	}();
	return path;
}

std::atomic<pid_t> g_child{0};
int run_helper(const std::vector<std::string>& args, const char* stdout_path, const char* stderr_path, const char* scratch_dir = nullptr)
{
	std::vector<char*> argv;
	for (const std::string& a : args) argv.push_back(const_cast<char*>(a.c_str()));
	argv.push_back(nullptr);
	posix_spawn_file_actions_t fa;
	posix_spawn_file_actions_init(&fa);
	posix_spawn_file_actions_addopen(&fa, 0, "/dev/null", O_RDONLY, 0);
	posix_spawn_file_actions_addopen(&fa, 1, stdout_path ? stdout_path : "/dev/null", O_WRONLY | O_CREAT | O_TRUNC, 0644);
	posix_spawn_file_actions_addopen(&fa, 2, stderr_path ? stderr_path : "/dev/null", O_WRONLY | O_CREAT | O_TRUNC, 0644);
#if defined(__GLIBC__) && __GLIBC_PREREQ(2, 34)
	posix_spawn_file_actions_addclosefrom_np(&fa, 3);
#endif
	pid_t pid = 0;
	std::vector<char*> envp;
	std::string scratch_var;
	for (char** e = environ; e && *e; e++) if (strncmp(*e, "ASTCENC_AMD_JITC_SCRATCH=", 25) != 0) envp.push_back(*e);
	if (scratch_dir) { scratch_var = std::string("ASTCENC_AMD_JITC_SCRATCH=") + scratch_dir; envp.push_back(const_cast<char*>(scratch_var.c_str())); }
	envp.push_back(nullptr);
	const int rc = posix_spawn(&pid, argv[0], &fa, nullptr, argv.data(), envp.data());
	posix_spawn_file_actions_destroy(&fa);
	if (rc != 0) return -1;
	g_child.store(pid);
	int status = 0;
	while (waitpid(pid, &status, 0) < 0 && errno == EINTR) { }
	g_child.store(0);
	return WIFEXITED(status) ? WEXITSTATUS(status) : -1;
}

std::string slurp(const std::string& path)
{
	std::string out;
	FILE* f = fopen(path.c_str(), "rb");
	if (!f) return out;
	char buf[65536];
	size_t n;
	while ((n = fread(buf, 1, sizeof(buf), f)) > 0) out.append(buf, n);
	fclose(f);
	return out;
}
bool spill(const std::string& path, const void* data, size_t n)
{
	FILE* f = fopen(path.c_str(), "wb");
	if (!f) return false;
	const bool ok = fwrite(data, 1, n, f) == n;
	return fclose(f) == 0 && ok;
}
std::string temp_dir()
{
	std::string base = cache_dir();
	if (!base.empty()) make_dirs(base); else { const char* t = getenv("TMPDIR"); base = t && *t ? t : "/tmp"; }
	std::string tmpl = base + "/jitXXXXXX";
	return mkdtemp(&tmpl[0]) ? tmpl : std::string();
}

const std::string& compiler_identity()
{
	static const std::string id = []() {
		const std::string helper = helper_path();
		if (!helper.empty())
		{
			const std::string dir = temp_dir();
			if (!dir.empty())
			{
				const std::string out = dir + "/identity.txt";
				const int rc = run_helper({ helper, "--identity" }, out.c_str(), nullptr);
				std::string text = rc == 0 ? slurp(out) : std::string();
				(void)unlink(out.c_str());
				(void)rmdir(dir.c_str());
				while (!text.empty() && (text.back() == '\n' || text.back() == ' ')) text.pop_back();
				if (!text.empty()) return "process " + text;
			}
		}
		std::string text = "inprocess ";
		struct link_map* lm = nullptr;
		if (rtc().handle && dlinfo(rtc().handle, RTLD_DI_LINKMAP, &lm) == 0 && lm && lm->l_name)
		{
			struct stat st;
			text += lm->l_name;
			if (stat(lm->l_name, &st) == 0) text += " " + std::to_string((long)st.st_size);
		}
		return text;
	}();
	return id;
}

long metadata_value(const std::vector<char>& code, const char* key)
{
	const size_t klen = strlen(key);
	for (size_t i = 0; i + klen + 1 < code.size(); i++)
	{
		if (memcmp(&code[i], key, klen) != 0) continue;
		const uint8_t* p = reinterpret_cast<const uint8_t*>(&code[i + klen]);
		const size_t left = code.size() - (i + klen);
		if (p[0] <= 0x7f) return p[0];
		if (p[0] == 0xcc && left > 1) return p[1];
		if (p[0] == 0xcd && left > 2) return (long)p[1] << 8 | p[2];
		if (p[0] == 0xce && left > 4) return (long)p[1] << 24 | (long)p[2] << 16 | (long)p[3] << 8 | p[4];
	}
	return -1;
}

bool acceptable(const std::vector<char>& code, long* vgprs, long* scratch)
{
	*vgprs = metadata_value(code, ".vgpr_count");
	*scratch = metadata_value(code, ".private_segment_fixed_size");
	return *vgprs >= 0 && *vgprs <= 128 && *scratch >= 0 && *scratch <= JIT_MAX_SCRATCH_BYTES;
}

}

struct JitKernel {
	std::string key;
	std::string name;
	std::string records;
	std::string unit;
	std::vector<std::string> options;
	std::vector<char> code;
	double seconds = 0.0;
	int refs = 0;
	JitState state = JIT_IDLE;
	void (*log)(const char*) = nullptr;
};

namespace {

struct Queue {
	std::mutex mu;
	std::condition_variable cv;
	std::deque<JitKernel*> pending;
	std::map<std::string, JitKernel*> by_key;
	std::thread worker;
	bool started = false, quit = false;
};
std::atomic<bool> g_compiling_in_process{false};
struct ExitGuard { ~ExitGuard(); };
Queue& queue() { static Queue* q = new Queue; static ExitGuard guard; (void)guard; return *q; }
ExitGuard::~ExitGuard()
{
	Queue& q = queue();
	std::unique_lock<std::mutex> g(q.mu);
	q.quit = true;
	q.pending.clear();
	q.cv.wait(g, [] { return !g_compiling_in_process.load(); });
}

void say(const JitKernel* k, const std::string& line) { if (k->log) k->log(line.c_str()); }

bool compile_in_process(JitKernel* k, std::string& diagnostics)
{
	const Rtc& r = rtc();
	if (!r.ok) { diagnostics = "no hipRTC library"; return false; }
	std::vector<const char*> texts, names;
	for (int i = 0; i < kHeaderCount; i++) { texts.push_back(kHeaders[i].text); names.push_back(kHeaders[i].name); }
	texts.push_back(k->records.c_str()); names.push_back("fixed_contexts.inc");
	hiprtcProgram prog = nullptr;
	if (r.create(&prog, k->unit.c_str(), "astc_compress_blocks_jit.hip", (int)texts.size(), texts.data(), names.data()) != HIPRTC_SUCCESS) return false;
	std::vector<const char*> opts;
	for (const std::string& o : k->options) opts.push_back(o.c_str());
	bool ok = r.compile(prog, (int)opts.size(), opts.data()) == HIPRTC_SUCCESS;
	if (!ok)
	{
		size_t n = 0;
		if (r.log_size(prog, &n) == HIPRTC_SUCCESS && n > 1) { diagnostics.resize(n); (void)r.log(prog, &diagnostics[0]); }
	}
	size_t bytes = 0;
	if (ok) ok = r.code_size(prog, &bytes) == HIPRTC_SUCCESS && bytes > 0;
	if (ok) { k->code.resize(bytes); ok = r.code(prog, k->code.data()) == HIPRTC_SUCCESS; }
	(void)r.destroy(&prog);
	return ok;
}

bool compile_in_helper(JitKernel* k, const std::string& helper, std::string& diagnostics)
{
	const std::string dir = temp_dir();
	if (dir.empty()) { diagnostics = "no scratch directory"; return false; }
	bool ok = true;
	std::vector<std::string> files;
	for (int i = 0; i < kHeaderCount && ok; i++)
	{
		files.push_back(dir + "/" + kHeaders[i].name);
		ok = spill(files.back(), kHeaders[i].text, (size_t)(kHeaders[i].end - kHeaders[i].text) - 1);
	}
	files.push_back(dir + "/fixed_contexts.inc");
	ok = ok && spill(files.back(), k->records.data(), k->records.size());
	files.push_back(dir + "/unit.hip");
	ok = ok && spill(files.back(), k->unit.data(), k->unit.size());
	const std::string cache = cache_dir();
	if (!cache.empty()) make_dirs(cache);
	const std::string out = cache.empty() ? dir + "/out.hsaco" : cache + "/" + k->key + ".hsaco", err = dir + "/stderr.txt";
	if (ok)
	{
		std::vector<std::string> args = { helper, dir + "/unit.hip", out };
		for (const std::string& o : k->options) args.push_back(o);
		args.push_back("-I" + dir);
		ok = run_helper(args, nullptr, err.c_str(), cache.empty() ? nullptr : dir.c_str()) == 0;
		if (!ok) diagnostics = slurp(err);
	}
	if (ok)
	{
		const std::string code = slurp(out);
		k->code.assign(code.begin(), code.end());
		ok = !k->code.empty();
	}
	for (const std::string& f : files) (void)unlink(f.c_str());
	if (cache.empty()) (void)unlink(out.c_str());
	(void)unlink(err.c_str());
	(void)rmdir(dir.c_str());
	return ok;
}

bool compile_now(JitKernel* k)
{
	const auto t0 = std::chrono::steady_clock::now();
	const std::string helper = helper_path();
	std::string diagnostics;
	if (helper.empty()) g_compiling_in_process.store(true);
	bool ok = helper.empty() ? compile_in_process(k, diagnostics) : compile_in_helper(k, helper, diagnostics);
	if (helper.empty()) { g_compiling_in_process.store(false); queue().cv.notify_all(); }
	k->seconds = std::chrono::duration<double>(std::chrono::steady_clock::now() - t0).count();
	if (!ok)
	{
		k->code.clear();
		say(k, "run-time build " + k->name + " failed to compile: " + diagnostics.substr(0, 600));
		return false;
	}
	long vgprs = 0, scratch = 0;
	if (!acceptable(k->code, &vgprs, &scratch))
	{
		say(k, "run-time build " + k->name + " refused: " + std::to_string(vgprs) + " VGPRs, " + std::to_string(scratch) + " bytes of scratch (compiler: " + compiler_identity() + "); the generic build stays");
		k->code.clear();
		return false;
	}
	const std::string dir = cache_dir();
	if (!dir.empty() && helper.empty())
	{
		make_dirs(dir);
		const std::string path = dir + "/" + k->key + ".hsaco";
		const std::string tpath = path + ".tmp" + std::to_string((long)getpid());
		if (spill(tpath, k->code.data(), k->code.size())) (void)rename(tpath.c_str(), path.c_str());
		else (void)unlink(tpath.c_str());
	}
	char line[256];
	snprintf(line, sizeof(line), " compiled in %.1f s (%zu bytes, %ld VGPRs, %ld bytes of scratch, %s)", k->seconds, k->code.size(), vgprs, scratch, helper.empty() ? "in process" : "compiler process");
	say(k, "run-time build " + k->name + line);
	return true;
}

bool load_cached(JitKernel* k)
{
	const std::string dir = cache_dir();
	if (dir.empty()) return false;
	FILE* f = fopen((dir + "/" + k->key + ".hsaco").c_str(), "rb");
	if (!f) return false;
	std::vector<char> data;
	char buf[65536];
	size_t n;
	while ((n = fread(buf, 1, sizeof(buf), f)) > 0) data.insert(data.end(), buf, buf + n);
	fclose(f);
	if (data.size() < 64 || memcmp(data.data(), "\177ELF", 4) != 0) return false;
	k->code.swap(data);
	return true;
}

void worker_main()
{
	Queue& q = queue();
	std::unique_lock<std::mutex> g(q.mu);
	for (;;)
	{
		q.cv.wait(g, [&] { return q.quit || !q.pending.empty(); });
		if (q.quit) return;
		JitKernel* k = q.pending.front();
		q.pending.pop_front();
		k->state = JIT_COMPILING;
		k->refs++;
		g.unlock();
		const bool ok = compile_now(k);
		g.lock();
		k->state = ok ? JIT_READY : JIT_FAILED;
		q.cv.notify_all();
		if (--k->refs == 0) { q.by_key.erase(k->key); delete k; }
	}
}

void start_locked(Queue& q, JitKernel* k)
{
	if (k->state != JIT_IDLE) return;
	k->state = JIT_QUEUED;
	q.pending.push_back(k);
	if (!q.started) { q.started = true; q.worker = std::thread(worker_main); }
	q.cv.notify_all();
}

}

bool jit_write_records(const char* path, const void* layout, size_t layout_bytes, const DeviceConfig& cfg_in, const TableRoot& root)
{
	if (layout_bytes != sizeof(LdsLayout)) return false;
	LdsLayout L;
	memcpy(&L, layout, sizeof(L));
	DeviceConfig cfg = cfg_in;
	cfg.debug_dup_stage = 0;
	const std::string text = records_text(L, cfg, root);
	return spill(path, text.data(), text.size());
}

JitMode jit_mode_from_environment()
{
	const char* e = getenv("ASTCENC_AMD_JIT");
	if (!e || !*e || strcmp(e, "lazy") == 0) return JIT_LAZY;
	if (strcmp(e, "off") == 0 || strcmp(e, "0") == 0) return JIT_OFF;
	if (strcmp(e, "eager") == 0 || strcmp(e, "async") == 0) return JIT_EAGER;
	if (strcmp(e, "sync") == 0) return JIT_SYNC;
	return JIT_LAZY;
}

JitKernel* jit_acquire(const void* layout, size_t layout_bytes, const DeviceConfig& cfg_in, const TableRoot& root, bool hdr, const char* arch,
                       void (*log)(const char*))
{
	if (layout_bytes != sizeof(LdsLayout) || (helper_path().empty() && !rtc().ok)) return nullptr;
	LdsLayout L;
	memcpy(&L, layout, sizeof(L));
	DeviceConfig cfg = cfg_in;
	cfg.debug_dup_stage = 0;
	JitKernel* k = new JitKernel;
	k->log = log;
	k->records = records_text(L, cfg, root);
	k->unit = std::string("#define ASTC_VARIANT v_jit\n") + (hdr ? "#define ASTC_ENABLE_HDR 1\n" : "#define ASTC_ENABLE_HDR 0\n") +
	          (root.texel_count <= 64 ? "#define ASTC_TEXELS_LE_64 1\n" : "#define ASTC_FIXED_OPAQUE_TEXEL_COUNT 1\n") +
	          "#define ASTC_FIXED_CONTEXT 1\n"
	          "#define ASTC_KERNEL_NAME astc_compress_blocks_jit\n#define ASTC_KERNEL_LINKAGE extern \"C\"\n#include \"kernel_device.h\"\n";
	std::string a = arch && *arch ? arch : "gfx950";
	a = a.substr(0, a.find(':'));
	k->options = { "--offload-arch=" + a, "-O3", "-std=c++17", "-ffp-contract=off", "-fhip-fp32-correctly-rounded-divide-sqrt", "-fno-math-errno",
	               "-fno-slp-vectorize", "-Wno-unused-function" };
	if (const char* more = getenv("ASTCENC_AMD_JIT_OPTIONS"))
	{
		std::string word;
		for (const char* p = more;; p++)
		{
			if (*p == ' ' || *p == 0) { if (!word.empty()) k->options.push_back(word); word.clear(); if (!*p) break; }
			else word.push_back(*p);
		}
	}
	uint64_t h = 14695981039346656037ull;
	for (int i = 0; i < kHeaderCount; i++) h = fnv1a(h, kHeaders[i].text, (size_t)(kHeaders[i].end - kHeaders[i].text));
	h = fnv1a(h, k->records.data(), k->records.size());
	h = fnv1a(h, k->unit.data(), k->unit.size());
	for (const std::string& o : k->options) h = fnv1a(h, o.data(), o.size() + 1);
	h = fnv1a(h, compiler_identity().data(), compiler_identity().size());
	char hex[24];
	snprintf(hex, sizeof(hex), "%016llx", (unsigned long long)h);
	k->key = hex;
	k->name = std::string(JIT_ENTRY_POINT) + "_" + hex;

	Queue& q = queue();
	std::lock_guard<std::mutex> g(q.mu);
	auto it = q.by_key.find(k->key);
	if (it != q.by_key.end()) { delete k; it->second->refs++; return it->second; }
	if (load_cached(k))
	{
		long vgprs = 0, scratch = 0;
		if (acceptable(k->code, &vgprs, &scratch)) k->state = JIT_READY;
		else
		{
			say(k, "run-time build " + k->name + " in the disk cache refused: " + std::to_string(vgprs) + " VGPRs, " + std::to_string(scratch) + " bytes of scratch; the generic build stays");
			k->code.clear();
			k->state = JIT_FAILED;
		}
	}
	k->refs = 1;
	q.by_key[k->key] = k;
	return k;
}

void jit_release(JitKernel* k)
{
	if (!k) return;
	Queue& q = queue();
	std::lock_guard<std::mutex> g(q.mu);
	if (--k->refs != 0) return;
	if (k->state == JIT_QUEUED)
		for (auto it = q.pending.begin(); it != q.pending.end(); ++it) if (*it == k) { q.pending.erase(it); break; }
	q.by_key.erase(k->key);
	delete k;
}

void jit_start(JitKernel* k)
{
	if (!k) return;
	Queue& q = queue();
	std::lock_guard<std::mutex> g(q.mu);
	start_locked(q, k);
}

JitState jit_wait(JitKernel* k)
{
	if (!k) return JIT_FAILED;
	Queue& q = queue();
	std::unique_lock<std::mutex> g(q.mu);
	start_locked(q, k);
	q.cv.wait(g, [&] { return k->state == JIT_READY || k->state == JIT_FAILED || q.quit; });
	return k->state;
}

JitState jit_state(const JitKernel* k)
{
	if (!k) return JIT_FAILED;
	Queue& q = queue();
	std::lock_guard<std::mutex> g(q.mu);
	return k->state;
}

const void* jit_code(const JitKernel* k, size_t* bytes) { *bytes = k->code.size(); return k->code.data(); }
const char* jit_kernel_name(const JitKernel* k) { return k->name.c_str(); }
double jit_compile_seconds(const JitKernel* k) { return k->seconds; }

}
```

astc-encoder_amd/csrc/kernel_ldr.hip:

```cpp
#define ASTC_VARIANT v_ldr
#define ASTC_ENABLE_HDR 0
#define ASTC_KERNEL_NAME astc_compress_blocks_ldr
#define ASTC_PREPARE_NAME astc_kernel_prepare_ldr
#define ASTC_LAUNCH_NAME astc_kernel_launch_ldr
#include "kernel_impl.h"
```

astc-encoder_amd/csrc/kernel_ldr64.hip:

```cpp
#define ASTC_VARIANT v_ldr64
#define ASTC_ENABLE_HDR 0
#define ASTC_TEXELS_LE_64 1
#define ASTC_KERNEL_NAME astc_compress_blocks_ldr64
#define ASTC_PREPARE_NAME astc_kernel_prepare_ldr64
#define ASTC_LAUNCH_NAME astc_kernel_launch_ldr64
#include "kernel_impl.h"
```

astc-encoder_amd/csrc/kernel_ldr_6x6m.hip:

```cpp
#define ASTC_VARIANT v_ldr_6x6m
#define ASTC_ENABLE_HDR 0
#define ASTC_TEXELS_LE_64 1
#define ASTC_FIXED_CONTEXT 1
#define ASTC_FIXED_ldr_6x6_medium 1
#define ASTC_KERNEL_NAME astc_compress_blocks_ldr_6x6m
#define ASTC_PREPARE_NAME astc_kernel_prepare_ldr_6x6m
#define ASTC_LAUNCH_NAME astc_kernel_launch_ldr_6x6m
#include "kernel_impl.h"
```

astc-encoder_amd/csrc/kernel_ldr_8x8t.hip:

```cpp
#define ASTC_VARIANT v_ldr_8x8t
#define ASTC_ENABLE_HDR 0
#define ASTC_TEXELS_LE_64 1
#define ASTC_FIXED_CONTEXT 1
#define ASTC_FIXED_ldr_8x8_thorough 1
#define ASTC_KERNEL_NAME astc_compress_blocks_ldr_8x8t
#define ASTC_PREPARE_NAME astc_kernel_prepare_ldr_8x8t
#define ASTC_LAUNCH_NAME astc_kernel_launch_ldr_8x8t
#include "kernel_impl.h"
```

astc-encoder_amd/csrc/wave_block.h:

```cpp
#pragma once
#if !defined(__HIP_DEVICE_COMPILE__)
#include <stddef.h>
#include <stdio.h>
#include <stdlib.h>
#endif
#include "wave_ctx.h"
#include "wave_quad.h"
#include "wave_load.h"
#include "wave_ideal.h"
#include "wave_weights.h"
#include "wave_format.h"
#include "wave_color.h"
#include "wave_refine.h"
#include "wave_batch.h"
#include "wave_partition.h"
#include "wave_pack.h"

namespace astcd { inline namespace ASTC_VARIANT {

WV_FN void copy_scb(Scb& dst, const Scb& src)
{
	const uint32_t* s = reinterpret_cast<const uint32_t*>(&src);
	uint32_t* d = reinterpret_cast<uint32_t*>(&dst);
	WV_FOR(i, (int)(sizeof(Scb) / 4)) { d[i] = s[i]; }
// ... 829 lines not shown
	const PartView pv = part_view_lds(c, partition_count, partition_packed);
	if (dual)
	{
		WV_FOR(ch, 4)
		{
			int plane = ch == plane2_component ? 1 : 0;
			tr.rgbs[1][ch] = tr.ep0[plane][0][ch];
			tr.rgbs[2][ch] = tr.ep1[plane][0][ch];
		}
		WV_SYNC();
	}
	PROF_SCOPE(c, PS_FORMATS);
	if (partition_count == 1)
		compute_ideal_endpoint_formats(c, part_view_lds(c, 1, 0), dual ? &tr.rgbs[1] : tr.ep0[0], dual ? &tr.rgbs[2] : tr.ep1[0], start, end);
	else
		compute_ideal_endpoint_formats(c, pv, tr.ep0[0], tr.ep1[0], start, end);
	select_candidate_modes(c, partition_count, start, end);
}

WV_FN float stage_refine(int partition_count, int partition_packed, int plane2_component, float tune_errorval_threshold)
{
	const Ctx c = ctx_make();
	partition_count = wv_uniform(partition_count); partition_packed = wv_uniform(partition_packed);
	plane2_component = wv_uniform(plane2_component); tune_errorval_threshold = wv_uniform(tune_errorval_threshold);
	PROF_SCOPE(c, PS_X2);
	return refine_candidates(c, partition_count, partition_packed, plane2_component, tune_errorval_threshold);
}

__attribute__((always_inline)) WV_FN float compress_trial(const Ctx& c, bool dual, bool only_always, float tune_errorval_threshold,
                           int partition_count, int partition_packed, int plane2_component, int quant_limit)
{
	PROF_SCOPE(c, PS_X3);
	tune_errorval_threshold = wv_uniform(tune_errorval_threshold);
	TRACE_PUT(c, TR_PASS, (float)(partition_count * 64 + (dual ? 2 : 1) * 8 + (plane2_component + 1)));
#if defined(ASTC_TRACE)
	if (partition_count > 1) TRACE_PUT(c, TR_PARTITION_INDEX, (float)part_view(c, partition_count, partition_packed).h->partition_index);
#endif
	const int max_weight_quant = i_min((int)QUANT_32, quant_limit);
	const int max_decimation_modes = wv_uniform(only_always ? (int)c.root->decimation_mode_count_always : (int)c.root->decimation_mode_count_selected);
	const int ref_mask = (int)((1u << (max_weight_quant + 1)) - 1);
	int mode_start, mode_end;
	if (dual)
	{
		mode_start = wv_uniform((int)c.root->block_mode_count_1plane_selected);
		mode_end = wv_uniform((int)c.root->block_mode_count_1plane_2plane_selected);
	}
	else
	{
		mode_start = 0;
		mode_end = wv_uniform(only_always ? (int)c.root->block_mode_count_1plane_always : (int)c.root->block_mode_count_1plane_selected);
	}

	DUP_STAGE(c, DUP_IDEAL, stage_ideal(dual, partition_count, partition_packed, plane2_component));
	DUP_STAGE(c, DUP_DECIMATE, stage_decimate(dual ? 2 : 1, ref_mask, max_decimation_modes));
	DUP_STAGE(c, DUP_ANGULAR, stage_angular(dual, partition_count, plane2_component, max_decimation_modes, ref_mask, max_weight_quant));
	DUP_STAGE(c, DUP_MODES_FORMATS, {
	DUP_STAGE(c, DUP_MODES, stage_modes(partition_count, mode_start, mode_end, max_weight_quant, dual));
	stage_formats(dual, partition_count, partition_packed, plane2_component, mode_start, mode_end); });
	return wv_uniform(stage_refine(partition_count, partition_packed, dual ? plane2_component : -1, tune_errorval_threshold));
}

__attribute__((always_inline)) WV_FN float compress_block_1plane(const Ctx& c, bool only_always, float tune_errorval_threshold,
                                  int partition_count, int partition_packed, int quant_limit)
{
	return compress_trial(c, false, only_always, tune_errorval_threshold, partition_count, partition_packed, -1, quant_limit);
}

__attribute__((always_inline)) WV_FN float compress_block_2planes(const Ctx& c, float tune_errorval_threshold, int plane2_component, int quant_limit)
{
	return compress_trial(c, true, false, tune_errorval_threshold, 1, 0, plane2_component, quant_limit);
}

WV_FN float prepare_block_statistics(const Ctx& c)
{
	TrialInfo& tr = c.tr();
	const BlkInfo& blk = c.blk();
	const int T = c.T;

	WV_FOR(k, 15)
	{
		const int ca[15] = { 0, 0, 1, 2, 3, 0, 1, 2, 3, 0, 0, 0, 1, 1, 2 };
		const int cb[15] = { -1, -1, -1, -1, -1, 0, 1, 2, 3, 1, 2, 3, 2, 3, 3 };
		const float* da = c.data(ca[k]);
		const float* db = cb[k] >= 0 ? c.data(cb[k]) : da;
		float acc = 0.0f;
		for (int i = 0; i < T; i++)
		{
			float weight = hadd4(cw_of(blk, 0), cw_of(blk, 1), cw_of(blk, 2), cw_of(blk, 3)) / 4.0f;
			if (k == 0) acc += weight;
			else
			{
				float aw = da[i] * weight;
				if (cb[k] < 0) acc += aw;
				else acc += db[i] * aw;
			}
		}
		tr.fbox[k] = acc;
	}
	WV_SYNC();

	const float* s = tr.fbox;
	float weight_sum = s[0], rs = s[1], gs = s[2], bs = s[3], as = s[4];
	float rr_var = s[5], gg_var = s[6], bb_var = s[7], aa_var = s[8];
	float rg_cov = s[9], rb_cov = s[10], ra_cov = s[11], gb_cov = s[12], ga_cov = s[13], ba_cov = s[14];

	float rpt = 1.0f / f_max(weight_sum, 1e-7f);

	rr_var -= rs * (rs * rpt);
	rg_cov -= gs * (rs * rpt);
	rb_cov -= bs * (rs * rpt);
	ra_cov -= as * (rs * rpt);

	gg_var -= gs * (gs * rpt);
	gb_cov -= bs * (gs * rpt);
	ga_cov -= as * (gs * rpt);

	bb_var -= bs * (bs * rpt);
	ba_cov -= as * (bs * rpt);

	aa_var -= as * (as * rpt);

	rg_cov *= 1.0f / f_sqrt(rr_var * gg_var);
	rb_cov *= 1.0f / f_sqrt(rr_var * bb_var);
	ra_cov *= 1.0f / f_sqrt(rr_var * aa_var);
	gb_cov *= 1.0f / f_sqrt(gg_var * bb_var);
	ga_cov *= 1.0f / f_sqrt(gg_var * aa_var);
	ba_cov *= 1.0f / f_sqrt(bb_var * aa_var);

	if (f_isnan(rg_cov)) rg_cov = 1.0f;
	if (f_isnan(rb_cov)) rb_cov = 1.0f;
	if (f_isnan(ra_cov)) ra_cov = 1.0f;
	if (f_isnan(gb_cov)) gb_cov = 1.0f;
	if (f_isnan(ga_cov)) ga_cov = 1.0f;
	if (f_isnan(ba_cov)) ba_cov = 1.0f;

	float lowest_correlation = f_min(f_abs(rg_cov), f_abs(rb_cov));
	lowest_correlation = f_min(lowest_correlation, f_abs(ra_cov));
	lowest_correlation = f_min(lowest_correlation, f_abs(gb_cov));
	lowest_correlation = f_min(lowest_correlation, f_abs(ga_cov));
	lowest_correlation = f_min(lowest_correlation, f_abs(ba_cov));
	WV_SYNC();
	return lowest_correlation;
}

WV_OUT int stage_partition_order(int partition_count)
{
	const Ctx c = ctx_make_vector_tables();
	partition_count = wv_uniform(partition_count);
	PROF_SCOPE(c, PS_KMEANS);
	return partition_search_order(c, partition_count);
}
WV_FN void stage_partition_score(int partition_count, int search_limit)
{
	const Ctx c = ctx_make();
	partition_count = wv_uniform(partition_count); search_limit = wv_uniform(search_limit);
	PROF_SCOPE(c, PS_KMEANS);
	partition_search_score(c, partition_count, search_limit);
}
WV_OUT int stage_partition_select(int search_limit, int requested_trials)
{
	const Ctx c = ctx_make();
	search_limit = wv_uniform(search_limit); requested_trials = wv_uniform(requested_trials);
	PROF_SCOPE(c, PS_KMEANS);
	return partition_search_select(c, search_limit, requested_trials);
}

WV_FN int stage_partition_search(const Ctx& c, int partition_count, int requested_indices, int requested_trials)
{
	(void)c;
	int sequence_len;
	DUP_STAGE(c, DUP_PART_ORDER, sequence_len = wv_uniform(stage_partition_order(partition_count)));
	const int search_limit = i_min(requested_indices, sequence_len);
	DUP_STAGE(c, DUP_PART_SCORE, stage_partition_score(partition_count, search_limit));
	int found;
	DUP_STAGE(c, DUP_PART_SELECT, found = stage_partition_select(search_limit, i_min(search_limit, requested_trials)));
	return found;
}

WV_OUT float stage_block_statistics()
{
	const Ctx c = ctx_make();
	PROF_SCOPE(c, PS_STATS);
	return prepare_block_statistics(c);
}

__attribute__((always_inline)) WV_FN void search_block(const Ctx& c)
{
	const BlkInfo& blk = c.blk();
	const DeviceConfig& cfg = *c.cfg;
	Scb& scb = c.scb();
	const int T = c.T;

	bool block_is_l = blk_is_luminance(blk);
	float block_is_l_scale = block_is_l ? 1.0f / 1.5f : 1.0f;
	bool block_is_la = blk_is_luminancealpha(blk);
	float block_is_la_scale = block_is_la ? 1.0f / 1.05f : 1.0f;

	float error_weight_sum = hadd4(cw_of(blk, 0), cw_of(blk, 1), cw_of(blk, 2), cw_of(blk, 3)) * (float)T;
	const float error_threshold = wv_uniform(cfg.tune_db_limit * error_weight_sum * block_is_l_scale * block_is_la_scale);

	TRACE_PUT(c, TR_THRESHOLD, error_threshold);
	WV_ONE
	{
		scb.errorval = ERROR_CALC_DEFAULT;
		scb.block_type = SYM_BTYPE_ERROR;
		c.tr().staged_color_quant[0] = -1;
		c.tr().staged_color_quant[1] = -1;
		c.tr().eci1_valid = 0;
		c.tr().ideal_1p1p_valid = 0;
		c.tr().dirsum1_mask = 0;
	}
	WV_SYNC();

	float best_errorval_prev_pcount = ERROR_CALC_DEFAULT;
	const float errorval_overshoot = wv_uniform(1.0f / cfg.tune_mse_overshoot);
	const float trial_threshold = wv_uniform(error_threshold * errorval_overshoot);

	int start_trial = 1;
	if (cfg.tune_search_mode0_enable >= 0.85f && c.root->dim_z == 1) start_trial = 0;

	int quant_limit = QUANT_32;
	bool done = false;

	for (int i = start_trial; i < 2 && !done; i++)
	{
		const float errorval_mult = i == 0 ? 1.0f / cfg.tune_mse_overshoot : 1.0f;
		float errorval;
		DUP_STAGE(c, i == 0 ? DUP_TRIAL_A0 : DUP_TRIAL_A1, errorval = compress_block_1plane(c, i == 0, error_threshold * errorval_mult * errorval_overshoot, 1, 0, QUANT_32));
		WV_SYNC();
		if (scb.block_type != SYM_BTYPE_ERROR)
		{
			quant_limit = wv_uniform((int)c.block_mode(scb.block_mode).quant_mode);
		}
		best_errorval_prev_pcount = wv_uniform(f_min(best_errorval_prev_pcount, errorval));
		if (errorval < (error_threshold * errorval_mult)) done = true;
	}

	if (!done)
	{
		float lowest_correl;
		DUP_STAGE(c, DUP_STATS, lowest_correl = wv_uniform(stage_block_statistics()));
		TRACE_PUT(c, TR_LOWEST_CORREL, lowest_correl);
		bool block_skip_two_plane = lowest_correl > cfg.tune_2plane_early_out_limit_correlation;
		for (int i = 3; i >= 0 && !done; i--)
		{
			if (block_skip_two_plane) continue;
			if (blk.grayscale && i != 3) continue;
			if (is_constant_channel(blk, i)) continue;

			float errorval;
			DUP_STAGE(c, DUP_TRIAL_2PLANES, errorval = compress_block_2planes(c, trial_threshold, i, quant_limit));
			WV_SYNC();
			if (errorval > (best_errorval_prev_pcount * 1.85f)) break;
			if (errorval < error_threshold) done = true;
		}
	}

	if (!done)
	{
		const int max_partitions = wv_uniform((int)cfg.tune_partition_count_limit);
		for (int partition_count = 2; partition_count <= max_partitions && !done; partition_count++)
		{
			int requested_indices = wv_uniform((int)cfg.tune_partition_index_limit[partition_count - 2]);
			int requested_trials = wv_uniform((int)cfg.tune_partitioning_candidate_limit[partition_count - 2]);
			requested_trials = i_min(requested_trials, requested_indices);

			int actual_trials;
			actual_trials = wv_uniform(stage_partition_search(c, partition_count, requested_indices, requested_trials));
			LaneArray128 partition_indices;
			partition_indices.clear();
			{
				const PartScratch& ps = *reinterpret_cast<const PartScratch*>(c.part());
				WV_FOR64(i, actual_trials) { partition_indices.set(i, ps.best[i]); }
			}
			WV_SYNC();

			const float best_error_in_prev = best_errorval_prev_pcount;
			const float exit_threshold = wv_uniform(partition_count == 2 ? cfg.tune_partition_early_out_limit_factor[0]
			                           : partition_count == 3 ? cfg.tune_partition_early_out_limit_factor[1] : 0.0f);
			float best_error = ERROR_CALC_DEFAULT;

			for (int i = 0; i < actual_trials; i++)
			{
				float errorval;
				DUP_STAGE(c, DUP_TRIAL_2PARTITIONS + (partition_count - 2), errorval = compress_block_1plane(c, false, trial_threshold,
				                                       partition_count, partition_indices.get(i), quant_limit));
				WV_SYNC();
				best_error = wv_uniform(f_min(best_error, errorval));

				if (best_error > (best_error_in_prev * (exit_threshold * 1.85f))) { done = true; break; }
				if (errorval < error_threshold) { done = true; break; }
			}
			if (done) break;

			if (best_error > (best_error_in_prev * exit_threshold)) { done = true; break; }
			best_errorval_prev_pcount = best_error;
		}
	}

}

WV_FN void compress_block(const Ctx& c, uint8_t* out)
{
	bool constant_color;
	{
		const BlkInfo& blk = c.blk();
		constant_color = blk.data_min[0] == blk.data_max[0] && blk.data_min[1] == blk.data_max[1] &&
		                 blk.data_min[2] == blk.data_max[2] && blk.data_min[3] == blk.data_max[3];
	}
	if (!wv_uniform(constant_color)) search_block(c);

	WV_SYNC();
	WV_ONE
	{
		const Ctx ce = ctx_make();
		Scb& scb = ce.scb();
		const BlkInfo& blk = ce.blk();
		if (constant_color)
		{
			scb.partition_count = 0;
			if (ce.cfg->profile == 3 || ce.cfg->profile == 2)
			{
				scb.block_type = SYM_BTYPE_CONST_F16;
				for (int k = 0; k < 4; k++) scb.constant_color[k] = float_to_half(blk.origin[k]);
			}
			else
			{
				scb.block_type = SYM_BTYPE_CONST_U16;
				for (int k = 0; k < 4; k++)
				{
					float v = v_clamp(0.0f, 1.0f, blk.origin[k]) * 65535.0f;
					scb.constant_color[k] = (int)(v + 0.5f);
				}
			}
		}
		else if (scb.block_type == SYM_BTYPE_ERROR)
		{
			scb.block_type = SYM_BTYPE_CONST_U16;
			for (int k = 0; k < 4; k++)
			{
				float v = v_clamp(0.0f, 1.0f, blk.origin[k]) * 65535.0f;
				scb.constant_color[k] = (int)(v + 0.5f);
			}
		}
	}
	WV_SYNC();
	{
		const Ctx ce = ctx_make();
		PROF_SCOPE(ce, PS_X1);
		uint8_t* pcb = out + (size_t)wv_uniform(ce.blk().block_index) * 16;
		DUP_STAGE(ce, DUP_PHYSICAL, symbolic_to_physical(ce, ce.scb(), pcb));
	}
}

} }
```

astc-encoder_amd/csrc/wave_load.h:

```cpp
#pragma once
#include "wave_ctx.h"

namespace astcd { inline namespace ASTC_VARIANT {

WV_FN float float_to_lns(float a)
{
	int ai = float_as_int(a);
	int exp = ((int)((unsigned)ai >> 23) & 0xFF) - 126;
	float mant = int_as_float((ai & (int)0x807FFFFF) | 0x3F000000);

	bool mask_underflow_nan = !(a > (1.0f / 67108864.0f));
	bool mask_infinity = a >= 65536.0f;
	bool exp_lt_m13 = exp < -13;

	float a1a = a * 33554432.0f;
	float a1b = (mant - 0.5f) * 4096;
	int expb = exp + 14;

	a = exp_lt_m13 ? a1a : a1b;
	exp = exp_lt_m13 ? 0 : expb;

	bool a_lt_384 = a < 384.0f;
	bool a_lt_1408 = a <= 1408.0f;

	float a2a = a * (4.0f / 3.0f);
	float a2b = a + 128.0f;
	float a2c = (a + 512.0f) * (4.0f / 5.0f);

	a = a2c;
	a = a_lt_1408 ? a2b : a;
	a = a_lt_384 ? a2a : a;

	a = a + ((float)exp * 2048.0f) + 1.0f;

	a = mask_infinity ? 65535.0f : a;
	a = mask_underflow_nan ? 0.0f : a;
	return a;
}

WV_FN int lns_to_sf16(int p)
{
	int mc = p & 0x7FF;
	int ec = (int)((unsigned)p >> 11);
	int mt;
	if (mc < 512) mt = mc * 3;
	else if (mc < 1536) mt = mc * 4 - 512;
	else mt = mc * 5 - 2048;
	int res = (ec << 10) | (int)((unsigned)mt >> 3);
	return i_min(res, 0x7BFF);
}

WV_FN void load_block(const Ctx& c, const ImageDesc& img, unsigned int bx, unsigned int by, unsigned int bz)
{
	const int T = c.T;
	const int dim_x = c.root->dim_x;
	const unsigned int plane_texels = (unsigned)dim_x * (unsigned)c.root->dim_y;
	const bool volume = c.root->dim_z > 1;
	BlkInfo& blk = c.blk();
	const int profile = c.cfg->profile;
	float* dr = c.data(0); float* dg = c.data(1); float* db = c.data(2); float* da = c.data(3);

	const bool fast = img.use_fast_load != 0;
	const int rgb_lns = (kHdr && (profile == 3  || profile == 2 )) ? 1 : 0;
	const int a_lns = (kHdr && profile == 3) ? 1 : 0;

	WV_FOR_T(t, T)
	{
		unsigned int tz = volume ? (unsigned)t / plane_texels : 0u;
		unsigned int trem = (unsigned)t - tz * plane_texels;
		unsigned int ty = trem / (unsigned)dim_x;
		unsigned int tx = trem - ty * (unsigned)dim_x;
		unsigned int xi = bx * (unsigned)dim_x + tx;
		unsigned int yi = by * (unsigned)c.root->dim_y + ty;
		unsigned int zi = bz * (unsigned)c.root->dim_z + tz;
		xi = xi < img.dim_x - 1 ? xi : img.dim_x - 1;
		yi = yi < img.dim_y - 1 ? yi : img.dim_y - 1;
		zi = zi < img.dim_z - 1 ? zi : img.dim_z - 1;
		if (fast && img.fast_load_slice0) zi = 0;
		size_t base = (size_t)4 * ((size_t)img.dim_x * ((size_t)img.dim_y * zi + yi) + xi);

		float v[6];
		if (img.data_type == 0)
		{
			uint32_t px = *reinterpret_cast<const uint32_t*>(static_cast<const uint8_t*>(img.data) + base);
			float r = (float)(px & 0xFF), g = (float)((px >> 8) & 0xFF), b = (float)((px >> 16) & 0xFF), a = (float)(px >> 24);
			if (fast)
			{
				dr[t] = r * (65535.0f / 255.0f);
				dg[t] = g * (65535.0f / 255.0f);
				db[t] = b * (65535.0f / 255.0f);
				da[t] = a * (65535.0f / 255.0f);
				continue;
			}
			v[0] = r / 255.0f; v[1] = g / 255.0f; v[2] = b / 255.0f; v[3] = a / 255.0f;
		}
		else if (img.data_type == 1)
		{
			const uint16_t* p = static_cast<const uint16_t*>(img.data) + base;
			v[0] = half_to_float(p[0]); v[1] = half_to_float(p[1]); v[2] = half_to_float(p[2]); v[3] = half_to_float(p[3]);
		}
		else
		{
			const float* p = static_cast<const float*>(img.data) + base;
			v[0] = p[0]; v[1] = p[1]; v[2] = p[2]; v[3] = p[3];
		}

		v[4] = 0.0f; v[5] = 1.0f;
		float s[4];
		for (int k = 0; k < 4; k++) s[k] = v[img.swz[k] < 6 ? img.swz[k] : 4];

		for (int k = 0; k < 4; k++)
		{
			float unorm = v_clamp(0.0f, 65535.0f, s[k] * 65535.0f);
			bool use_lns = k < 3 ? rgb_lns : a_lns;
			float out = use_lns ? float_to_lns(s[k]) : unorm;
			c.data(k)[t] = out;
		}
	}
	WV_FOR(t, c.Tp - T)
	{
		for (int k = 0; k < 4; k++) c.data(k)[T + t] = 0.0f;
	}
	WV_SYNC();

	WV_FOR(k, 4)
	{
		const float* d = c.data(k);
		float mn = 1e38f, mx = -1e38f, mean = 0.0f;
		float scale = 1.0f / (float)T;
		for (int t = 0; t < T; t++)
		{
			float v = d[t];
			mn = mn < v ? mn : v;
			mx = mx > v ? mx : v;
			if (fast) mean += v; else mean += v * scale;
		}
		if (fast) mean = mean / (float)T;
		blk.data_min[k] = mn;
		blk.data_max[k] = mx;
		blk.data_mean[k] = mean;
		blk.cw[k] = c.cfg->cw[k];

		float e = d[0];
		float origin = e / 65535.0f;
		bool use_lns = !fast && (k < 3 ? rgb_lns : a_lns);
		if (use_lns)
		{
			origin = half_to_float((uint16_t)lns_to_sf16((int)e));
		}
		blk.origin[k] = origin;

		if (k == 0)
		{
			bool gray = true;
			for (int t = 0; t < T; t++)
			{
				gray = gray && (dr[t] == dg[t]) && (dr[t] == db[t]);
			}
			blk.grayscale = gray ? 1 : 0;
			blk.rgb_lns = fast ? 0 : rgb_lns;
			blk.alpha_lns = fast ? 0 : a_lns;
		}
	}
	WV_SYNC();

	if (c.cfg->flags & (1u << 2))
	{
		WV_ONE
		{
			float alpha_scale = blk.data_max[3] * (1.0f / 65535.0f);
			blk.cw[0] = c.cfg->cw[0] * alpha_scale;
			blk.cw[1] = c.cfg->cw[1] * alpha_scale;
			blk.cw[2] = c.cfg->cw[2] * alpha_scale;
			blk.cw[3] = c.cfg->cw[3];
		}
		WV_SYNC();
	}
}

WV_FN bool block_has_visible_alpha(const Ctx& c, const ImageDesc& img, unsigned int bx, unsigned int by)
{
	const int dim_x = c.root->dim_x, dim_y = c.root->dim_y;
	const unsigned int r = img.a_scale_radius;
	const float footprint = (float)((size_t)(dim_x + 2 * (r - 1)) * (size_t)(dim_y + 2 * (r - 1)));
	const float threshold = 0.9f / (255.0f * footprint);
	bool seen = false;
	WV_FOR_T(t, c.T)
	{
		unsigned int ty = (unsigned)t / (unsigned)dim_x;
		unsigned int tx = (unsigned)t - ty * (unsigned)dim_x;
		unsigned int xi = bx * (unsigned)dim_x + tx, yi = by * (unsigned)dim_y + ty;
		if (xi < img.dim_x && yi < img.dim_y && img.alpha_avg[(size_t)yi * img.dim_x + xi] > threshold) seen = true;
	}
	return wv_any(seen);
}

WV_FN void load_transparent_block(const Ctx& c)
{
	BlkInfo& blk = c.blk();
	WV_ONE
	{
		for (int k = 0; k < 4; k++)
		{
			blk.origin[k] = 0.0f; blk.data_min[k] = 0.0f; blk.data_mean[k] = 0.0f; blk.data_max[k] = 0.0f;
			blk.cw[k] = c.cfg->cw[k];
		}
		blk.grayscale = 1;
		blk.rgb_lns = 0;
		blk.alpha_lns = 0;
	}
	WV_SYNC();
}

} }
```

astc-encoder_amd/csrc/wave_pack.h:

```cpp
#pragma once
#include "wave_ctx.h"

namespace astcd { inline namespace ASTC_VARIANT {

struct Btq { uint8_t bits, trits, quints; };

WV_FN Btq btq_of(int q)
{
	const uint8_t bits[21]   = { 1,0,2,0,1,3,1,2,4,2,3,5,3,4,6,4,5,7,5,6,8 };
	const uint8_t kind[21]   = { 0,1,0,2,1,0,2,1,0,2,1,0,2,1,0,2,1,0,2,1,0 };
	Btq b; b.bits = bits[q]; b.trits = kind[q] == 1; b.quints = kind[q] == 2;
	return b;
}

WV_FN unsigned int ise_bitcount(unsigned int count, int q)
{
	Btq b = btq_of(q);
	unsigned int total = b.bits * count;
	if (b.trits)  total += (8 * count + 4) / 5;
	if (b.quints) total += (7 * count + 2) / 3;
	return total;
}

WV_FN unsigned int quant_level_count(int q)
{
	const uint16_t lv[21] = { 2,3,4,5,6,8,10,12,16,20,24,32,40,48,64,80,96,128,160,192,256 };
	return lv[q];
}

WV_FN void bits_or(uint32_t* words, uint32_t value, uint32_t count, uint32_t offset)
{
	value &= count >= 32u ? 0xFFFFFFFFu : (1u << count) - 1u;
	const uint32_t w = offset >> 5, sh = offset & 31u;
	const uint32_t lo = value << sh, hi = sh ? value >> (32u - sh) : 0u;
#if WV_DEVICE
	if (lo) __hip_atomic_fetch_or(words + w, lo, __ATOMIC_RELAXED, __HIP_MEMORY_SCOPE_WORKGROUP);
	if (hi) __hip_atomic_fetch_or(words + w + 1, hi, __ATOMIC_RELAXED, __HIP_MEMORY_SCOPE_WORKGROUP);
#else
	words[w] |= lo;
	if (hi) words[w + 1] |= hi;
#endif
}

WV_FN void encode_ise_lanes(const Ctx& c, int quant, int count, const uint8_t* sym, uint32_t* words, uint32_t base)
{
	const Btq b = btq_of(quant);
	const uint32_t bits = b.bits, low_mask = (1u << bits) - 1u;
	const uint8_t* trit_tab = c.table(c.root->off_integer_of_trits);
	const uint8_t* quint_tab = c.table(c.root->off_integer_of_quints);
	WV_FOR64(s, count)
	{
		const uint32_t v = sym[s];
		if (b.trits)
		{
			const uint32_t g = ((uint32_t)s * 13u) >> 6, k = (uint32_t)s - g * 5u;
			uint32_t t[5];
			for (uint32_t j = 0; j < 5; j++) t[j] = (int)(g * 5u + j) < count ? (uint32_t)(sym[g * 5u + j] >> bits) : 0u;
			const uint32_t word = trit_tab[(((t[4] * 3 + t[3]) * 3 + t[2]) * 3 + t[1]) * 3 + t[0]];
			const uint32_t place = (0x75420u >> (4u * k)) & 0xFu;
			const uint32_t width = (0x12122u >> (4u * k)) & 0xFu;
			bits_or(words, (v & low_mask) | (((word >> place) & ((1u << width) - 1u)) << bits), bits + width, base + g * (5u * bits + 8u) + k * bits + place);
		}
		else if (b.quints)
		{
			const uint32_t g = ((uint32_t)s * 43u) >> 7, k = (uint32_t)s - g * 3u;
			uint32_t q[3];
			for (uint32_t j = 0; j < 3; j++) q[j] = (int)(g * 3u + j) < count ? (uint32_t)(sym[g * 3u + j] >> bits) : 0u;
			const uint32_t word = quint_tab[(q[2] * 5 + q[1]) * 5 + q[0]];
			const uint32_t place = (0x530u >> (4u * k)) & 0xFu;
			const uint32_t width = (0x223u >> (4u * k)) & 0xFu;
			bits_or(words, (v & low_mask) | (((word >> place) & ((1u << width) - 1u)) << bits), bits + width, base + g * (3u * bits + 7u) + k * bits + place);
		}
		else
		{
			bits_or(words, v, bits, base + (uint32_t)s * bits);
		}
	}
}

WV_FN uint32_t bit_reverse32(uint32_t v)
{
#if WV_DEVICE
	return __builtin_bitreverse32(v);
#else
	v = ((v >> 1) & 0x55555555u) | ((v & 0x55555555u) << 1);
	v = ((v >> 2) & 0x33333333u) | ((v & 0x33333333u) << 2);
	v = ((v >> 4) & 0x0F0F0F0Fu) | ((v & 0x0F0F0F0Fu) << 4);
	v = ((v >> 8) & 0x00FF00FFu) | ((v & 0x00FF00FFu) << 8);
	return (v >> 16) | (v << 16);
#endif
}

WV_FN void symbolic_to_physical(const Ctx& c, const Scb& scb, uint8_t* pcb_out)
{
	uint32_t* block = reinterpret_cast<uint32_t*>(c.lds + c.L->uni);
	uint32_t* stream = block + 8;
	uint8_t* weight_sym = reinterpret_cast<uint8_t*>(block + 16);
	uint8_t* colour_sym = weight_sym + 64;
	WV_FOR(k, 16) { block[k] = 0u; }
	WV_SYNC();

	const int block_type = wv_uniform((int)scb.block_type);
	if (block_type == SYM_BTYPE_CONST_U16 || block_type == SYM_BTYPE_CONST_F16)
	{
		WV_ONE
		{
			uint32_t* out = reinterpret_cast<uint32_t*>(pcb_out);
			out[0] = block_type == SYM_BTYPE_CONST_U16 ? 0xFFFFFDFCu : 0xFFFFFFFCu;
			out[1] = 0xFFFFFFFFu;
			out[2] = (uint32_t)(scb.constant_color[0] & 0xFFFF) | ((uint32_t)(scb.constant_color[1] & 0xFFFF) << 16);
			out[3] = (uint32_t)(scb.constant_color[2] & 0xFFFF) | ((uint32_t)(scb.constant_color[3] & 0xFFFF) << 16);
		}
		return;
	}

	const int partition_count = wv_uniform((int)scb.partition_count);
	const BlockMode& bm = c.block_mode(wv_uniform((int)scb.block_mode));
	const int weight_count = wv_uniform((int)c.dec_info(bm.decimation_mode).weight_count);
	const int wq = wv_uniform((int)bm.quant_mode);
	const bool dual = wv_uniform((int)bm.is_dual_plane) != 0;
	const int real_weight_count = dual ? 2 * weight_count : weight_count;
	const int bits_for_weights = (int)ise_bitcount((unsigned)real_weight_count, wq);
	const int colour_quant = wv_uniform((int)scb.quant_mode);

	{
		const QuantXfer& qat = c.qxfer(wq);
		const float top = (float)quant_level_count(wq) - 1.0f;
		WV_FOR64(s, real_weight_count)
		{
			const int i = dual ? s >> 1 : s, plane = dual ? s & 1 : 0;
			const float uqw = (float)scb.weights[i + plane * PLANE2_OFFSET];
			const int level = (int)((uqw / 64.0f) * top + 0.5f);
			weight_sym[s] = qat.scramble_map[level];
		}
	}
	int value_count = 0;
	for (int p = 0; p < partition_count; p++) value_count += 2 * (scb.color_formats[p] >> 2) + 2;
	value_count = wv_uniform(value_count);
	{
		const uint8_t* pack_table = c.table(c.root->off_color_uquant_to_pquant) + (colour_quant - QUANT_6) * 256;
		WV_FOR64(v, value_count)
		{
			int p = 0, j = v;
			for (int q = 0; q < 3; q++)
			{
				const int n = 2 * (scb.color_formats[q] >> 2) + 2;
				if (p == q && q + 1 < partition_count && j >= n) { j -= n; p++; }
			}
			colour_sym[v] = pack_table[scb.color_values[p][j]];
		}
	}
	WV_SYNC();

	encode_ise_lanes(c, wq, real_weight_count, weight_sym, stream, 0u);
	encode_ise_lanes(c, colour_quant, value_count, colour_sym, block, partition_count == 1 ? 17u : 29u);

	WV_ONE
	{
		bits_or(block, bm.mode_index, 11, 0);
		bits_or(block, (uint32_t)(partition_count - 1), 2, 11);
		int below_weights_pos = 128 - bits_for_weights;
		if (partition_count > 1)
		{
			const uint32_t seed = reinterpret_cast<const PartitionHeader*>(c.part_rec(partition_count, scb.partition_index))->partition_index;
			bits_or(block, seed, 10, 13);
			if (scb.color_formats_matched)
			{
				bits_or(block, (uint32_t)scb.color_formats[0] << 2, 6, 23);
			}
			else
			{
				int low_class = 4;
				for (int i = 0; i < partition_count; i++) low_class = i_min(scb.color_formats[i] >> 2, low_class);
				if (low_class == 3) low_class = 2;
				uint32_t encoded = (uint32_t)(low_class + 1);
				for (int i = 0; i < partition_count; i++)
				{
					encoded |= (uint32_t)((scb.color_formats[i] >> 2) - low_class) << (2 + i);
					encoded |= (uint32_t)(scb.color_formats[i] & 3) << (2 + partition_count + 2 * i);
				}
				const int high_size = 3 * partition_count - 4;
				bits_or(block, encoded & 0x3Fu, 6, 23);
				bits_or(block, encoded >> 6, (uint32_t)high_size, (uint32_t)(128 - bits_for_weights - high_size));
				below_weights_pos -= high_size;
			}
		}
		else
		{
			bits_or(block, scb.color_formats[0], 4, 13);
		}
		if (dual) bits_or(block, (uint32_t)scb.plane2_component, 2, (uint32_t)(below_weights_pos - 2));
	}
	WV_SYNC();

	WV_FOR(d, 4)
	{
		reinterpret_cast<uint32_t*>(pcb_out)[d] = block[d] | bit_reverse32(stream[3 - d]);
	}
}

} }
```

Baseline: 220.4.

## Launch a resident-sized persistent grid that pulls blocks from per-XCD atomic tickets

When the block count exceeds the number of resident workgroups, the kernel is launched with a grid sized from occupancy (CUs times workgroups per CU). Each persistent workgroup loops, taking block indices from per-XCD atomic ticket counters and stealing from other XCDs' counters once its own runs dry. This removes the per-workgroup launch and teardown cost and the tail imbalance, at the price of a memset, an event dependency and a global atomic per block. Kernel arguments are now read through the kernarg pointer so they can be reloaded inside the loop, and the JIT build adds the -sink-insts-to-avoid-spills option.

```diff
diff --git a/astc-encoder_amd/csrc/astc_tables.h b/astc-encoder_amd/csrc/astc_tables.h
--- a/astc-encoder_amd/csrc/astc_tables.h
+++ b/astc-encoder_amd/csrc/astc_tables.h
@@ -254,6 +254,7 @@
 	uint32_t dim_z, blocks_z;
 	uint32_t fast_load_slice0;
 	const uint32_t* list;
+	uint32_t* tickets;
 };
 
 struct ImageSetEntryDesc {
diff --git a/astc-encoder_amd/csrc/backend.h b/astc-encoder_amd/csrc/backend.h
--- a/astc-encoder_amd/csrc/backend.h
+++ b/astc-encoder_amd/csrc/backend.h
@@ -82,6 +82,7 @@
 	img.alpha_avg = nullptr;
 	img.a_scale_radius = job.a_scale_radius;
 	img.list = job.device_list;
+	img.tickets = nullptr;
 	return img;
 }
 
@@ -194,20 +195,26 @@
 	void* stream;
 	unsigned long long* d_prof;
 	const ImageSetTable* d_set;
+	uint32_t grid = 0;
 };
 
 int astc_kernel_prepare_ldr(const TableRoot& root, const DeviceConfig& cfg, uint32_t* lds_bytes, void* layout_out, uint32_t* layout_bytes);
 int astc_kernel_prepare_hdr(const TableRoot& root, const DeviceConfig& cfg, uint32_t* lds_bytes, void* layout_out, uint32_t* layout_bytes);
 int astc_kernel_launch_ldr(const KernelLaunch& k);
 int astc_kernel_launch_hdr(const KernelLaunch& k);
+int astc_kernel_occupancy_ldr(uint32_t lds_bytes, int* workgroups_per_cu);
+int astc_kernel_occupancy_hdr(uint32_t lds_bytes, int* workgroups_per_cu);
 int astc_kernel_prepare_ldr64(const TableRoot& root, const DeviceConfig& cfg, uint32_t* lds_bytes, void* layout_out, uint32_t* layout_bytes);
 int astc_kernel_prepare_hdr64(const TableRoot& root, const DeviceConfig& cfg, uint32_t* lds_bytes, void* layout_out, uint32_t* layout_bytes);
 int astc_kernel_launch_ldr64(const KernelLaunch& k);
 int astc_kernel_launch_hdr64(const KernelLaunch& k);
+int astc_kernel_occupancy_ldr64(uint32_t lds_bytes, int* workgroups_per_cu);
+int astc_kernel_occupancy_hdr64(uint32_t lds_bytes, int* workgroups_per_cu);
 constexpr int ASTC_PREPARE_NOT_THIS_CONTEXT = -1;
 #define ASTC_DECLARE_KERNEL_VARIANT(tag) \
 	int astc_kernel_prepare_##tag(const TableRoot& root, const DeviceConfig& cfg, uint32_t* lds_bytes, void* layout_out, uint32_t* layout_bytes); \
-	int astc_kernel_launch_##tag(const KernelLaunch& k);
+	int astc_kernel_launch_##tag(const KernelLaunch& k); \
+	int astc_kernel_occupancy_##tag(uint32_t lds_bytes, int* workgroups_per_cu);
 ASTC_DECLARE_KERNEL_VARIANT(ldr_6x6m)
 ASTC_DECLARE_KERNEL_VARIANT(ldr_8x8t)
 ASTC_DECLARE_KERNEL_VARIANT(hdr_6x6m)
diff --git a/astc-encoder_amd/csrc/backend_hip.hip b/astc-encoder_amd/csrc/backend_hip.hip
--- a/astc-encoder_amd/csrc/backend_hip.hip
+++ b/astc-encoder_amd/csrc/backend_hip.hip
@@ -1,4 +1,5 @@
 #include "backend.h"
+#include "block_tickets.h"
 #include "kernel_jit.h"
 #include "mip_resample.h"
 
@@ -66,6 +67,9 @@
 	hipModule_t jit_module = nullptr;
 	hipFunction_t jit_fn = nullptr;
 	bool jit_tried = false;
+	uint32_t* d_tickets = nullptr;
+	uint32_t resident_lib = 0, resident_jit = 0;
+	hipEvent_t ev_tickets = nullptr;
 };
 
 struct Backend {
@@ -157,15 +161,16 @@
 	bool fixed, hdr, small;
 	int (*prepare)(const TableRoot&, const DeviceConfig&, uint32_t*, void*, uint32_t*);
 	int (*launch)(const KernelLaunch&);
+	int (*occupancy)(uint32_t, int*);
 };
 const KernelVariant kernel_variants[] = {
-	{ "astc_compress_blocks_ldr_6x6m", true, false, true, astc_kernel_prepare_ldr_6x6m, astc_kernel_launch_ldr_6x6m },
-	{ "astc_compress_blocks_ldr_8x8t", true, false, true, astc_kernel_prepare_ldr_8x8t, astc_kernel_launch_ldr_8x8t },
-	{ "astc_compress_blocks_hdr_6x6m", true, true, true, astc_kernel_prepare_hdr_6x6m, astc_kernel_launch_hdr_6x6m },
-	{ "astc_compress_blocks_ldr64", false, false, true, astc_kernel_prepare_ldr64, astc_kernel_launch_ldr64 },
-	{ "astc_compress_blocks_hdr64", false, true, true, astc_kernel_prepare_hdr64, astc_kernel_launch_hdr64 },
-	{ "astc_compress_blocks_ldr", false, false, false, astc_kernel_prepare_ldr, astc_kernel_launch_ldr },
-	{ "astc_compress_blocks_hdr", false, true, false, astc_kernel_prepare_hdr, astc_kernel_launch_hdr },
+	{ "astc_compress_blocks_ldr_6x6m", true, false, true, astc_kernel_prepare_ldr_6x6m, astc_kernel_launch_ldr_6x6m, astc_kernel_occupancy_ldr_6x6m },
+	{ "astc_compress_blocks_ldr_8x8t", true, false, true, astc_kernel_prepare_ldr_8x8t, astc_kernel_launch_ldr_8x8t, astc_kernel_occupancy_ldr_8x8t },
+	{ "astc_compress_blocks_hdr_6x6m", true, true, true, astc_kernel_prepare_hdr_6x6m, astc_kernel_launch_hdr_6x6m, astc_kernel_occupancy_hdr_6x6m },
+	{ "astc_compress_blocks_ldr64", false, false, true, astc_kernel_prepare_ldr64, astc_kernel_launch_ldr64, astc_kernel_occupancy_ldr64 },
+	{ "astc_compress_blocks_hdr64", false, true, true, astc_kernel_prepare_hdr64, astc_kernel_launch_hdr64, astc_kernel_occupancy_hdr64 },
+	{ "astc_compress_blocks_ldr", false, false, false, astc_kernel_prepare_ldr, astc_kernel_launch_ldr, astc_kernel_occupancy_ldr },
+	{ "astc_compress_blocks_hdr", false, true, false, astc_kernel_prepare_hdr, astc_kernel_launch_hdr, astc_kernel_occupancy_hdr },
 };
 int kernel_prepare(Backend* b, uint32_t* lds_bytes, void* layout_out, uint32_t* layout_bytes)
 {
@@ -190,11 +195,63 @@
 	{
 		KernelLaunch a = k;
 		void* args[] = { &a.d_tab, &a.img, &a.d_out, &a.first, &a.count, &a.d_prof, &a.d_set };
-		return (int)hipModuleLaunchKernel(s->jit_fn, k.count, 1, 1, 64, 1, 1, k.lds_bytes, static_cast<hipStream_t>(k.stream), args, nullptr);
+		return (int)hipModuleLaunchKernel(s->jit_fn, k.img.tickets ? k.grid : k.count, 1, 1, 64, 1, 1, k.lds_bytes, static_cast<hipStream_t>(k.stream), args, nullptr);
 	}
 	return kernel_variants[b->variant].launch(k);
 }
 
+long compress_grid_from_env()
+{
+	static const long v = []() {
+		const char* e = getenv("ASTCENC_AMD_COMPRESS_GRID");
+		if (!e || !*e) return -1L;
+		char* end = nullptr;
+		const long n = strtol(e, &end, 10);
+		return end != e && n >= 0 && n <= 0x7fffffffL ? n : -1L;
+	}();
+	return v;
+}
+
+constexpr uint32_t RESIDENT_UNKNOWN = 0xFFFFFFFFu;
+uint32_t compress_grid(const Backend* b, DeviceSlot* s)
+{
+	uint32_t& resident = s->jit_fn ? s->resident_jit : s->resident_lib;
+	if (resident) return resident == RESIDENT_UNKNOWN ? 0 : resident;
+	int cus = 0, per_cu = 0;
+	hipError_t e = hipDeviceGetAttribute(&cus, hipDeviceAttributeMultiprocessorCount, s->device);
+	if (e == hipSuccess)
+		e = s->jit_fn ? hipModuleOccupancyMaxActiveBlocksPerMultiprocessor(&per_cu, s->jit_fn, 64, b->lds_bytes)
+		              : (hipError_t)kernel_variants[b->variant].occupancy(b->lds_bytes, &per_cu);
+	if (e != hipSuccess || cus <= 0 || per_cu <= 0)
+	{
+		(void)hipGetLastError();
+		log_msg("occupancy of %s on device %d unknown: one workgroup per block", s->jit_fn ? "the run-time build" : kernel_variants[b->variant].name, s->device);
+		resident = RESIDENT_UNKNOWN;
+		return 0;
+	}
+	resident = (uint32_t)cus * (uint32_t)per_cu;
+	log_msg("%s on device %d: %u workgroups resident (%d CUs x %d); a launch of more blocks draws them from tickets",
+	        s->jit_fn ? "the run-time build" : kernel_variants[b->variant].name, s->device, resident, cus, per_cu);
+	return resident;
+}
+
+int tickets_arm(DeviceSlot* s, KernelLaunch& k, uint32_t grid)
+{
+	const hipStream_t stream = static_cast<hipStream_t>(k.stream);
+	HIP_TRY(hipStreamWaitEvent(stream, s->ev_tickets, 0), return 2);
+	HIP_TRY(hipMemsetAsync(s->d_tickets, 0, TICKET_BUFFER_BYTES, stream), return 2);
+	k.img.tickets = s->d_tickets;
+	k.grid = grid;
+	return 0;
+}
+int tickets_launched(DeviceSlot* s, const KernelLaunch& k)
+{
+	const hipStream_t stream = static_cast<hipStream_t>(k.stream);
+	HIP_TRY(hipEventRecord(s->ev_tickets, stream), return 2);
+	return 0;
+}
+
+constexpr uint32_t JIT_SELF_CHECK_GRID = 288;
 bool jit_self_check(Backend* b, DeviceSlot* s, hipFunction_t fn)
 {
 	const uint32_t bsx = b->root.dim_x, bsy = b->root.dim_y, bsz = b->root.dim_z;
@@ -249,8 +306,10 @@
 		k.d_out = d_out;
 		ok = ok && kernel_variants[b->variant].launch(k) == 0;
 		k.d_out = d_out + nblocks * 16;
+		ok = ok && tickets_arm(s, k, JIT_SELF_CHECK_GRID) == 0;
 		void* args[] = { &k.d_tab, &k.img, &k.d_out, &k.first, &k.count, &k.d_prof, &k.d_set };
-		ok = ok && hipModuleLaunchKernel(fn, k.count, 1, 1, 64, 1, 1, k.lds_bytes, s->stream, args, nullptr) == hipSuccess;
+		ok = ok && hipModuleLaunchKernel(fn, k.grid, 1, 1, 64, 1, 1, k.lds_bytes, s->stream, args, nullptr) == hipSuccess;
+		ok = ok && tickets_launched(s, k) == 0;
 		ok = ok && hipMemcpyAsync(out.data(), d_out, out.size(), hipMemcpyDeviceToHost, s->stream) == hipSuccess;
 		ok = ok && hipStreamSynchronize(s->stream) == hipSuccess;
 		if (!ok) (void)hipGetLastError();
@@ -319,6 +378,8 @@
 	if (s->d_adaptive) (void)hipFree(s->d_adaptive);
 	for (hipEvent_t e : s->ev_adapt) if (e) (void)hipEventDestroy(e);
 	if (s->d_prof) (void)hipFree(s->d_prof);
+	if (s->d_tickets) (void)hipFree(s->d_tickets);
+	if (s->ev_tickets) (void)hipEventDestroy(s->ev_tickets);
 	for (int i = 0; i < 2; i++) { if (s->h_in[i]) (void)hipHostFree(s->h_in[i]); if (s->h_out[i]) (void)hipHostFree(s->h_out[i]); }
 	for (hipEvent_t e : { s->ev_copy[0], s->ev_copy[1], s->ev_band, s->ev_done[0], s->ev_done[1], s->ev_done[2], s->ev_out[0], s->ev_out[1], s->ev0, s->ev1, s->ev_gen })
 		if (e) (void)hipEventDestroy(e);
@@ -449,6 +510,8 @@
 	SLOT_TRY(hipEventCreate(&s->ev0), 2);
 	SLOT_TRY(hipEventCreate(&s->ev1), 2);
 	SLOT_TRY(hipEventCreate(&s->ev_gen), 2);
+	SLOT_TRY(hipEventCreateWithFlags(&s->ev_tickets, hipEventDisableTiming), 2);
+	SLOT_TRY(hipMalloc(reinterpret_cast<void**>(&s->d_tickets), TICKET_BUFFER_BYTES), 1);
 #if defined(ASTC_PROFILE)
 	enum { PS_COUNT = 40 };
 	SLOT_TRY(hipMalloc(&s->d_prof, 2 * PS_COUNT * sizeof(unsigned long long)), 1);
@@ -761,8 +824,14 @@
 		if (L.before_launch && L.before_launch(first, n) != 0) return 2;
 		KernelLaunch k = L.k;
 		k.first = (uint32_t)first; k.count = (uint32_t)n;
+		const long forced = compress_grid_from_env();
+		uint32_t grid = 0;
+		if (forced > 0) grid = (uint32_t)((size_t)forced < n ? (size_t)forced : n);
+		else if (forced < 0) { const uint32_t resident = compress_grid(b, s); if (resident && n > resident) grid = resident; }
+		if (grid && tickets_arm(s, k, grid) != 0) return 2;
 		int lrc = kernel_launch(b, s, k);
 		if (lrc != 0) { log_msg("kernel launch failed (hip error %d)", lrc); return 2; }
+		if (grid && tickets_launched(s, k) != 0) return 2;
 		L.launched = first + n;
 		if (L.after_launch)
 		{
diff --git a/astc-encoder_amd/csrc/block_tickets.h b/astc-encoder_amd/csrc/block_tickets.h
--- /dev/null
+++ b/astc-encoder_amd/csrc/block_tickets.h
@@ -0,0 +1,26 @@
+#pragma once
+
+#if defined(__HIPCC__)
+#define ASTC_TICKET_FN __host__ __device__ inline
+#else
+#define ASTC_TICKET_FN inline
+#endif
+
+namespace astcd {
+
+constexpr unsigned int TICKET_HEADS = 8;
+constexpr unsigned int TICKET_HEAD_STRIDE_WORDS = 16;
+constexpr unsigned int TICKET_BUFFER_BYTES = TICKET_HEADS * TICKET_HEAD_STRIDE_WORDS * 4;
+
+ASTC_TICKET_FN unsigned int ticket_head_word(unsigned int x) { return x * TICKET_HEAD_STRIDE_WORDS; }
+
+ASTC_TICKET_FN unsigned int ticket_head_count(unsigned int n, unsigned int x)
+{
+	return n > x ? (n - x - 1u) / TICKET_HEADS + 1u : 0u;
+}
+
+ASTC_TICKET_FN unsigned int ticket_index(unsigned int t, unsigned int x) { return TICKET_HEADS * t + x; }
+
+ASTC_TICKET_FN unsigned int ticket_head_after(unsigned int home, unsigned int dry) { return (home + dry) % TICKET_HEADS; }
+
+}
diff --git a/astc-encoder_amd/csrc/kernel_device.h b/astc-encoder_amd/csrc/kernel_device.h
--- a/astc-encoder_amd/csrc/kernel_device.h
+++ b/astc-encoder_amd/csrc/kernel_device.h
@@ -1,6 +1,7 @@
 #pragma once
 #include "wave_block.h"
 #include "image_set.h"
+#include "block_tickets.h"
 
 #ifndef ASTC_KERNEL_LINKAGE
 #define ASTC_KERNEL_LINKAGE
@@ -30,13 +31,33 @@
 	return g * group + (r % 8u) * XCD_SET_RUN + r / 8u;
 }
 
-ASTC_KERNEL_LINKAGE __global__ void __launch_bounds__(64, ASTC_WAVES_PER_EU) __attribute__((amdgpu_waves_per_eu(ASTC_WAVES_PER_EU)))
-ASTC_KERNEL_NAME(const uint8_t* __restrict__ tab, ImageDesc img,
-                 uint8_t* __restrict__ out, uint32_t first_block, uint32_t num_blocks, unsigned long long* prof,
-                 const ImageSetTable* __restrict__ set)
+struct CompressKernelArgs {
+	const uint8_t* tab;
+	ImageDesc img;
+	uint8_t* out;
+	uint32_t first_block, num_blocks;
+	unsigned long long* prof;
+	const ImageSetTable* set;
+};
+
+__attribute__((always_inline)) __device__ inline CompressKernelArgs compress_kernel_args()
 {
+	uintptr_t args_bits = reinterpret_cast<uintptr_t>(__builtin_amdgcn_kernarg_segment_ptr());
+	asm volatile("" : "+s"(args_bits));
+	return image_set_record<CompressKernelArgs>((const __attribute__((address_space(4))) uint32_t*)args_bits);
+}
+
+__attribute__((always_inline)) __device__ inline void compress_launch_index(uint32_t index)
+{
+	WV_LANE_SCOPE;
 	typedef const __attribute__((address_space(4))) uint8_t* constant_bytes;
-	uint32_t b = (set ? xcd_block_remap_runs(blockIdx.x, num_blocks) : xcd_block_remap(blockIdx.x, num_blocks)) + first_block;
+	const CompressKernelArgs a = compress_kernel_args();
+	ImageDesc img = a.img;
+	uint8_t* __restrict__ out = a.out;
+	const uint8_t* __restrict__ tab = a.tab;
+	unsigned long long* prof = a.prof;
+	const ImageSetTable* __restrict__ set = a.set;
+	uint32_t b = (set ? xcd_block_remap_runs(index, a.num_blocks) : xcd_block_remap(index, a.num_blocks)) + a.first_block;
 	if (img.list)
 	{
 		b = reinterpret_cast<const __attribute__((address_space(4))) uint32_t*>(reinterpret_cast<uintptr_t>(img.list))[b];
@@ -110,4 +131,56 @@
 	compress_block(c, out);
 }
 
+__device__ inline uint32_t home_xcd()
+{
+	uint32_t x;
+	asm("s_getreg_b32 %0, hwreg(HW_REG_XCC_ID, 0, 4)" : "=s"(x));
+	return x % TICKET_HEADS;
 }
+
+ASTC_KERNEL_LINKAGE __global__ void __launch_bounds__(64, ASTC_WAVES_PER_EU) __attribute__((amdgpu_waves_per_eu(ASTC_WAVES_PER_EU)))
+ASTC_KERNEL_NAME(const uint8_t* __restrict__ tab, ImageDesc img,
+                 uint8_t* __restrict__ out, uint32_t first_block, uint32_t num_blocks, unsigned long long* prof,
+                 const ImageSetTable* __restrict__ set)
+{
+	typedef __attribute__((address_space(1))) uint32_t* global_words;
+	const uint32_t home = img.tickets ? home_xcd() : 0u;
+	uint32_t dry = 0;
+	for (;;)
+	{
+		const CompressKernelArgs a = compress_kernel_args();
+		uint32_t index = blockIdx.x;
+		if (a.img.tickets)
+		{
+			const global_words heads = (global_words)reinterpret_cast<uintptr_t>(a.img.tickets);
+			for (;;)
+			{
+				if (dry == TICKET_HEADS) return;
+				const uint32_t x = ticket_head_after(home, dry);
+				uint32_t t = 0;
+				WV_ONE t = __hip_atomic_fetch_add(heads + ticket_head_word(x), 1u, __ATOMIC_RELAXED, __HIP_MEMORY_SCOPE_AGENT);
+				t = wv_uniform(t);
+				if (t < ticket_head_count(a.num_blocks, x)) { index = ticket_index(t, x); break; }
+				dry++;
+			}
+		}
+		compress_launch_index(index);
+		if (!compress_kernel_args().img.tickets) return;
+		WV_SYNC();
+	}
+}
+
+template <class A, class B> struct same_type { static constexpr bool value = false; };
+template <class A> struct same_type<A, A> { static constexpr bool value = true; };
+static_assert(same_type<decltype(&ASTC_KERNEL_NAME),
+                        void (*)(decltype(CompressKernelArgs::tab), decltype(CompressKernelArgs::img), decltype(CompressKernelArgs::out),
+                                 decltype(CompressKernelArgs::first_block), decltype(CompressKernelArgs::num_blocks),
+                                 decltype(CompressKernelArgs::prof), decltype(CompressKernelArgs::set))>::value,
+              "CompressKernelArgs does not mirror the kernel's parameter list");
+static_assert(sizeof(ImageDesc) % 8 == 0 && __builtin_offsetof(CompressKernelArgs, tab) == 0 && __builtin_offsetof(CompressKernelArgs, img) == 8 &&
+              __builtin_offsetof(CompressKernelArgs, out) == 8 + sizeof(ImageDesc) && __builtin_offsetof(CompressKernelArgs, first_block) == 16 + sizeof(ImageDesc) &&
+              __builtin_offsetof(CompressKernelArgs, num_blocks) == 20 + sizeof(ImageDesc) && __builtin_offsetof(CompressKernelArgs, prof) == 24 + sizeof(ImageDesc) &&
+              __builtin_offsetof(CompressKernelArgs, set) == 32 + sizeof(ImageDesc) && sizeof(CompressKernelArgs) == 40 + sizeof(ImageDesc),
+              "CompressKernelArgs has members, padding or an order that the kernel's argument segment does not");
+
+}
diff --git a/astc-encoder_amd/csrc/kernel_hdr.hip b/astc-encoder_amd/csrc/kernel_hdr.hip
--- a/astc-encoder_amd/csrc/kernel_hdr.hip
+++ b/astc-encoder_amd/csrc/kernel_hdr.hip
@@ -3,4 +3,5 @@
 #define ASTC_KERNEL_NAME astc_compress_blocks_hdr
 #define ASTC_PREPARE_NAME astc_kernel_prepare_hdr
 #define ASTC_LAUNCH_NAME astc_kernel_launch_hdr
+#define ASTC_OCCUPANCY_NAME astc_kernel_occupancy_hdr
 #include "kernel_impl.h"
diff --git a/astc-encoder_amd/csrc/kernel_hdr64.hip b/astc-encoder_amd/csrc/kernel_hdr64.hip
--- a/astc-encoder_amd/csrc/kernel_hdr64.hip
+++ b/astc-encoder_amd/csrc/kernel_hdr64.hip
@@ -4,4 +4,5 @@
 #define ASTC_KERNEL_NAME astc_compress_blocks_hdr64
 #define ASTC_PREPARE_NAME astc_kernel_prepare_hdr64
 #define ASTC_LAUNCH_NAME astc_kernel_launch_hdr64
+#define ASTC_OCCUPANCY_NAME astc_kernel_occupancy_hdr64
 #include "kernel_impl.h"
diff --git a/astc-encoder_amd/csrc/kernel_hdr_6x6m.hip b/astc-encoder_amd/csrc/kernel_hdr_6x6m.hip
--- a/astc-encoder_amd/csrc/kernel_hdr_6x6m.hip
+++ b/astc-encoder_amd/csrc/kernel_hdr_6x6m.hip
@@ -6,4 +6,5 @@
 #define ASTC_KERNEL_NAME astc_compress_blocks_hdr_6x6m
 #define ASTC_PREPARE_NAME astc_kernel_prepare_hdr_6x6m
 #define ASTC_LAUNCH_NAME astc_kernel_launch_hdr_6x6m
+#define ASTC_OCCUPANCY_NAME astc_kernel_occupancy_hdr_6x6m
 #include "kernel_impl.h"
diff --git a/astc-encoder_amd/csrc/kernel_impl.h b/astc-encoder_amd/csrc/kernel_impl.h
--- a/astc-encoder_amd/csrc/kernel_impl.h
+++ b/astc-encoder_amd/csrc/kernel_impl.h
@@ -31,13 +31,21 @@
 #if defined(ASTC_LDS_PAD_ENV)
 	static const unsigned pad = getenv("ASTC_LDS_PAD") ? (unsigned)atoi(getenv("ASTC_LDS_PAD")) : 0u;
 	if (pad) (void)hipFuncSetAttribute(reinterpret_cast<const void*>(ASTC_KERNEL_NAME), hipFuncAttributeMaxDynamicSharedMemorySize, (int)(k.lds_bytes + pad));
-	hipLaunchKernelGGL(ASTC_KERNEL_NAME, dim3(k.count), dim3(64), k.lds_bytes + pad, static_cast<hipStream_t>(k.stream),
+	hipLaunchKernelGGL(ASTC_KERNEL_NAME, dim3(k.img.tickets ? k.grid : k.count), dim3(64), k.lds_bytes + pad, static_cast<hipStream_t>(k.stream),
 	                   k.d_tab, k.img, k.d_out, k.first, k.count, k.d_prof, k.d_set);
 	return (int)hipGetLastError();
 #endif
-	hipLaunchKernelGGL(ASTC_KERNEL_NAME, dim3(k.count), dim3(64), k.lds_bytes, static_cast<hipStream_t>(k.stream),
+	hipLaunchKernelGGL(ASTC_KERNEL_NAME, dim3(k.img.tickets ? k.grid : k.count), dim3(64), k.lds_bytes, static_cast<hipStream_t>(k.stream),
 	                   k.d_tab, k.img, k.d_out, k.first, k.count, k.d_prof, k.d_set);
 	return (int)hipGetLastError();
 }
 
+int ASTC_OCCUPANCY_NAME(uint32_t lds_bytes, int* workgroups_per_cu)
+{
+#if defined(ASTC_LDS_PAD_ENV)
+	if (getenv("ASTC_LDS_PAD")) lds_bytes += (unsigned)atoi(getenv("ASTC_LDS_PAD"));
+#endif
+	return (int)hipOccupancyMaxActiveBlocksPerMultiprocessor(workgroups_per_cu, reinterpret_cast<const void*>(ASTC_KERNEL_NAME), 64, lds_bytes);
 }
+
+}
diff --git a/astc-encoder_amd/csrc/kernel_jit.cpp b/astc-encoder_amd/csrc/kernel_jit.cpp
--- a/astc-encoder_amd/csrc/kernel_jit.cpp
+++ b/astc-encoder_amd/csrc/kernel_jit.cpp
@@ -44,6 +44,7 @@
 ASTC_EMBED(astc_src_wave_partition, "wave_partition.h")
 ASTC_EMBED(astc_src_wave_pack, "wave_pack.h")
 ASTC_EMBED(astc_src_image_set, "image_set.h")
+ASTC_EMBED(astc_src_block_tickets, "block_tickets.h")
 
 extern char** environ;
 
@@ -60,7 +61,7 @@
 	{ "wave_color.h", astc_src_wave_color, astc_src_wave_color_end }, { "wave_color_hdr.h", astc_src_wave_color_hdr, astc_src_wave_color_hdr_end },
 	{ "wave_refine.h", astc_src_wave_refine, astc_src_wave_refine_end }, { "wave_batch.h", astc_src_wave_batch, astc_src_wave_batch_end },
 	{ "wave_partition.h", astc_src_wave_partition, astc_src_wave_partition_end }, { "wave_pack.h", astc_src_wave_pack, astc_src_wave_pack_end },
-	{ "image_set.h", astc_src_image_set, astc_src_image_set_end },
+	{ "image_set.h", astc_src_image_set, astc_src_image_set_end }, { "block_tickets.h", astc_src_block_tickets, astc_src_block_tickets_end },
 };
 constexpr int kHeaderCount = (int)(sizeof(kHeaders) / sizeof(kHeaders[0]));
 constexpr long JIT_MAX_SCRATCH_BYTES = 32;
@@ -506,7 +507,8 @@
 	std::string a = arch && *arch ? arch : "gfx950";
 	a = a.substr(0, a.find(':'));
 	k->options = { "--offload-arch=" + a, "-O3", "-std=c++17", "-ffp-contract=off", "-fhip-fp32-correctly-rounded-divide-sqrt", "-fno-math-errno",
-	               "-fno-slp-vectorize", "-Wno-unused-function" };
+	               "-fno-slp-vectorize", "-Wno-unused-function",
+	               "-mllvm", "-sink-insts-to-avoid-spills" };
 	if (const char* more = getenv("ASTCENC_AMD_JIT_OPTIONS"))
 	{
 		std::string word;
diff --git a/astc-encoder_amd/csrc/kernel_ldr.hip b/astc-encoder_amd/csrc/kernel_ldr.hip
--- a/astc-encoder_amd/csrc/kernel_ldr.hip
+++ b/astc-encoder_amd/csrc/kernel_ldr.hip
@@ -3,4 +3,5 @@
 #define ASTC_KERNEL_NAME astc_compress_blocks_ldr
 #define ASTC_PREPARE_NAME astc_kernel_prepare_ldr
 #define ASTC_LAUNCH_NAME astc_kernel_launch_ldr
+#define ASTC_OCCUPANCY_NAME astc_kernel_occupancy_ldr
 #include "kernel_impl.h"
diff --git a/astc-encoder_amd/csrc/kernel_ldr64.hip b/astc-encoder_amd/csrc/kernel_ldr64.hip
--- a/astc-encoder_amd/csrc/kernel_ldr64.hip
+++ b/astc-encoder_amd/csrc/kernel_ldr64.hip
@@ -4,4 +4,5 @@
 #define ASTC_KERNEL_NAME astc_compress_blocks_ldr64
 #define ASTC_PREPARE_NAME astc_kernel_prepare_ldr64
 #define ASTC_LAUNCH_NAME astc_kernel_launch_ldr64
+#define ASTC_OCCUPANCY_NAME astc_kernel_occupancy_ldr64
 #include "kernel_impl.h"
diff --git a/astc-encoder_amd/csrc/kernel_ldr_6x6m.hip b/astc-encoder_amd/csrc/kernel_ldr_6x6m.hip
--- a/astc-encoder_amd/csrc/kernel_ldr_6x6m.hip
+++ b/astc-encoder_amd/csrc/kernel_ldr_6x6m.hip
@@ -6,4 +6,5 @@
 #define ASTC_KERNEL_NAME astc_compress_blocks_ldr_6x6m
 #define ASTC_PREPARE_NAME astc_kernel_prepare_ldr_6x6m
 #define ASTC_LAUNCH_NAME astc_kernel_launch_ldr_6x6m
+#define ASTC_OCCUPANCY_NAME astc_kernel_occupancy_ldr_6x6m
 #include "kernel_impl.h"
diff --git a/astc-encoder_amd/csrc/kernel_ldr_8x8t.hip b/astc-encoder_amd/csrc/kernel_ldr_8x8t.hip
--- a/astc-encoder_amd/csrc/kernel_ldr_8x8t.hip
+++ b/astc-encoder_amd/csrc/kernel_ldr_8x8t.hip
@@ -6,4 +6,5 @@
 #define ASTC_KERNEL_NAME astc_compress_blocks_ldr_8x8t
 #define ASTC_PREPARE_NAME astc_kernel_prepare_ldr_8x8t
 #define ASTC_LAUNCH_NAME astc_kernel_launch_ldr_8x8t
+#define ASTC_OCCUPANCY_NAME astc_kernel_occupancy_ldr_8x8t
 #include "kernel_impl.h"
diff --git a/astc-encoder_amd/csrc/wave_block.h b/astc-encoder_amd/csrc/wave_block.h
--- a/astc-encoder_amd/csrc/wave_block.h
+++ b/astc-encoder_amd/csrc/wave_block.h
@@ -1155,6 +1155,7 @@
 
 WV_FN void compress_block(const Ctx& c, uint8_t* out)
 {
+	WV_LANE_SCOPE;
 	bool constant_color;
 	{
 		const BlkInfo& blk = c.blk();
@@ -1169,6 +1170,8 @@
 		const Ctx ce = ctx_make();
 		Scb& scb = ce.scb();
 		const BlkInfo& blk = ce.blk();
+		constant_color = blk.data_min[0] == blk.data_max[0] && blk.data_min[1] == blk.data_max[1] &&
+		                 blk.data_min[2] == blk.data_max[2] && blk.data_min[3] == blk.data_max[3];
 		if (constant_color)
 		{
 			scb.partition_count = 0;
diff --git a/astc-encoder_amd/csrc/wave_load.h b/astc-encoder_amd/csrc/wave_load.h
--- a/astc-encoder_amd/csrc/wave_load.h
+++ b/astc-encoder_amd/csrc/wave_load.h
@@ -52,6 +52,7 @@
 
 WV_FN void load_block(const Ctx& c, const ImageDesc& img, unsigned int bx, unsigned int by, unsigned int bz)
 {
+	WV_LANE_SCOPE;
 	const int T = c.T;
 	const int dim_x = c.root->dim_x;
 	const unsigned int plane_texels = (unsigned)dim_x * (unsigned)c.root->dim_y;
@@ -180,6 +181,7 @@
 
 WV_FN bool block_has_visible_alpha(const Ctx& c, const ImageDesc& img, unsigned int bx, unsigned int by)
 {
+	WV_LANE_SCOPE;
 	const int dim_x = c.root->dim_x, dim_y = c.root->dim_y;
 	const unsigned int r = img.a_scale_radius;
 	const float footprint = (float)((size_t)(dim_x + 2 * (r - 1)) * (size_t)(dim_y + 2 * (r - 1)));
@@ -197,6 +199,7 @@
 
 WV_FN void load_transparent_block(const Ctx& c)
 {
+	WV_LANE_SCOPE;
 	BlkInfo& blk = c.blk();
 	WV_ONE
 	{
diff --git a/astc-encoder_amd/csrc/wave_pack.h b/astc-encoder_amd/csrc/wave_pack.h
--- a/astc-encoder_amd/csrc/wave_pack.h
+++ b/astc-encoder_amd/csrc/wave_pack.h
@@ -44,6 +44,7 @@
 
 WV_FN void encode_ise_lanes(const Ctx& c, int quant, int count, const uint8_t* sym, uint32_t* words, uint32_t base)
 {
+	WV_LANE_SCOPE;
 	const Btq b = btq_of(quant);
 	const uint32_t bits = b.bits, low_mask = (1u << bits) - 1u;
 	const uint8_t* trit_tab = c.table(c.root->off_integer_of_trits);
@@ -93,6 +94,7 @@
 
 WV_FN void symbolic_to_physical(const Ctx& c, const Scb& scb, uint8_t* pcb_out)
 {
+	WV_LANE_SCOPE;
 	uint32_t* block = reinterpret_cast<uint32_t*>(c.lds + c.L->uni);
 	uint32_t* stream = block + 8;
 	uint8_t* weight_sym = reinterpret_cast<uint8_t*>(block + 16);
```

Result: faster. 233.1 (median of 6 runs) (+5.8%).
